# beltegeuse/rustlight

Measured on AMD Instinct MI355X. Metric: Msamples/s (paths/s) at 1080p x 128spp cbox, higher is better.
Workload: dtype f32

## Files before the change

### rustlight_amd/api.py

```python
from __future__ import annotations

import contextlib
import ctypes as C
import os
import time
from typing import Optional

import numpy as np

from . import abi
from . import scenes as S

_HERE = os.path.dirname(os.path.abspath(__file__))
LIB_PATH = os.path.join(_HERE, "lib", "librustlight_amd.so")

RL_OK = 0
RL_ERR_NO_DEVICE = -2
STRATEGY_ALL, STRATEGY_BSDF, STRATEGY_EMITTER = 0, 1, 2
STREAM_REFERENCE_ORDER, STREAM_PER_SAMPLE, STREAM_STRATIFIED = 0, 1, 2
PIPELINE_AUTO, PIPELINE_WAVEFRONT, PIPELINE_FUSED = 0, 1, 2
NUMERICS_EXACT, NUMERICS_FAST = 0, 1
LIGHT_ALL, LIGHT_SURFACE, LIGHT_VOLUME = 0, 1, 2
VPL_ALL, VPL_SURFACE, VPL_VOLUME = 0, 1, 2
LIGHT_STREAMS = ("reference", "per_path")
# ... 252 lines not shown
        for k, (w, h, rgb) in enumerate(sd.bitmaps):
            bitmaps[k].width, bitmaps[k].height, bitmaps[k].rgb = w, h, fp(rgb)
        d.bitmaps, d.n_bitmaps = bitmaps, len(sd.bitmaps)
        lights = (abi.LightDesc * max(1, len(sd.lights)))()
        for k, lt in enumerate(sd.lights):
            lights[k].kind = 0 if lt["type"] == "point" else 1
            lights[k].a = (C.c_float * 3)(*lt["a"])
            lights[k].intensity = (C.c_float * 3)(*lt["intensity"])
        d.lights, d.n_lights = lights, len(sd.lights)
        if sd.environment is not None:
            d.has_environment = 1
            d.environment_rgb = (C.c_float * 3)(*sd.environment)
        if sd.environment_map is not None:
            em = np.ascontiguousarray(sd.environment_map, np.float32); keep.append(em)
            d.env_map_width, d.env_map_height, d.env_map_rgb = em.shape[1], em.shape[0], abi.fptr(em)
        if sd.medium is not None:
            d.has_medium = 1
            d.sigma_a = (C.c_float * 3)(*sd.medium.sigma_a)
            d.sigma_s = (C.c_float * 3)(*sd.medium.sigma_s)
            d.phase_type, d.g = sd.medium.phase, sd.medium.g
        d.build_ats = int(bool(getattr(sd, "use_ats", False)))
        h = C.c_void_p()
        _check(lib().rl_scene_create_from_desc(C.byref(d), C.byref(h)))
        obj = cls.__new__(cls)
        obj.sd, obj.h = sd, h
        return obj

    @classmethod
    def load_pbrt(cls, path: str, use_shading_normals: bool = True) -> "Scene":
        h = C.c_void_p()
        _check(lib().rl_scene_load_pbrt(path.encode(), int(use_shading_normals), C.byref(h)))
        return cls(None, handle=h)

    @classmethod
    def load_mitsuba(cls, path: str, use_shading_normals: bool = True) -> "Scene":
        h = C.c_void_p()
        _check(lib().rl_scene_load_mitsuba(path.encode(), int(use_shading_normals), C.byref(h)))
        return cls(None, handle=h)

    @classmethod
    def load(cls, path: str, use_shading_normals: bool = True) -> "Scene":
        h = C.c_void_p()
        _check(lib().rl_scene_load(path.encode(), int(use_shading_normals), C.byref(h)))
        return cls(None, handle=h)

    def set_medium(self, sigma_a, sigma_s, phase=S.PHASE_ISOTROPIC, g=0.0):
        sa = np.asarray(sigma_a, dtype=np.float32)
        ss = np.asarray(sigma_s, dtype=np.float32)
        _check(lib().rl_scene_set_medium(self.h, abi.fptr(sa), abi.fptr(ss), phase, g))

    def __del__(self):
        try:
            lib().rl_scene_destroy(self.h)
        except Exception:
            pass

    @property
    def size(self):
        w, h = C.c_uint32(), C.c_uint32()
        _check(lib().rl_scene_image_size(self.h, C.byref(w), C.byref(h)))
        return w.value, h.value

    def counts(self):
        a, b, c = C.c_uint64(), C.c_uint64(), C.c_uint64()
        _check(lib().rl_scene_counts(self.h, C.byref(a), C.byref(b), C.byref(c)))
        return {"meshes": a.value, "triangles": b.value, "emitters": c.value}

    def debug_bvh(self):
        nn, npr = C.c_uint64(), C.c_uint64()
        _check(lib().rl_debug_bvh(self.h, C.byref(nn), C.byref(npr), None, None, None, None, None))
        boxes = np.zeros((nn.value, 6), np.float32)
        info = np.zeros(nn.value, np.uint64)
        count = np.zeros(nn.value, np.uint64)
        pm = np.zeros(npr.value, np.int32)
        pt = np.zeros(npr.value, np.int32)
        _check(lib().rl_debug_bvh(self.h, C.byref(nn), C.byref(npr), abi.fptr(boxes), abi.u64ptr(info), abi.u64ptr(count),
                                  pm.ctypes.data_as(C.POINTER(C.c_int32)), pt.ctypes.data_as(C.POINTER(C.c_int32))))
        return boxes, info, count, pm, pt

    def debug_emitters_cdf(self):
        n = C.c_uint64(0)
        L = lib()
        L.rl_debug_emitters_cdf.argtypes = [C.c_void_p, C.POINTER(C.c_uint64), C.POINTER(C.c_float)]
        _check(L.rl_debug_emitters_cdf(self.h, C.byref(n), None))
        out = np.zeros(n.value, np.float32)
        _check(L.rl_debug_emitters_cdf(self.h, C.byref(n), abi.fptr(out)))
        return out

    def debug_ats(self):
        L = lib()
        i32p = C.POINTER(C.c_int32)
        L.rl_debug_ats.argtypes = [C.c_void_p, C.POINTER(C.c_uint64), C.POINTER(C.c_float), C.POINTER(C.c_uint64), i32p, i32p]
        nn, nl = C.c_uint64(), C.c_uint64()
        _check(L.rl_debug_ats(self.h, C.byref(nn), None, C.byref(nl), None, None))
        nodes = np.zeros((nn.value, 16), np.float32); le = np.zeros(nl.value, np.int32); lp = np.zeros(nl.value, np.int32)
        _check(L.rl_debug_ats(self.h, C.byref(nn), abi.fptr(nodes), C.byref(nl), le.ctypes.data_as(i32p), lp.ctypes.data_as(i32p)))
        return nodes, le, lp

    def camera_ray(self, px, py):
        o = (C.c_float * 3)()
        d = (C.c_float * 3)()
        _check(lib().rl_debug_camera_ray(self.h, px, py, o, d))
        return np.array(o[:], np.float32), np.array(d[:], np.float32)


def path_params(spp=1, min_depth=0, max_depth=None, rr_depth=0, strategy=STRATEGY_ALL, single_scattering=False,
                stream_mode=STREAM_PER_SAMPLE, seed_variant=0, shard_index=0, shard_count=1, pool_slots=0, pipeline=0, sample_split=0, numerics=0) -> abi.PathParams:
    p = abi.PathParams()
    lib().rl_path_params_default(C.byref(p))
    p.spp = spp
    p.has_min_depth, p.min_depth = (0, 0) if min_depth is None else (1, min_depth)
    p.has_max_depth, p.max_depth = (0, 0) if max_depth is None else (1, max_depth)
    p.has_rr_depth, p.rr_depth = (0, 0) if rr_depth is None else (1, rr_depth)
    p.strategy = strategy
    p.single_scattering = int(single_scattering)
    p.stream_mode = stream_mode
    p.seed_variant = seed_variant
    p.shard_index, p.shard_count = shard_index, shard_count
    p.pool_slots = pool_slots
    p.pipeline = pipeline
    p.sample_split = sample_split
    p.numerics = numerics
    return p


class _ImageCalls:

    def _image_call(self, seeds, call, out=None):
        seeds = np.ascontiguousarray(seeds, dtype=np.uint64)
        st = abi.RenderStats()
        img = np.zeros((self.height, self.width, 3), dtype=np.float32) if out is None else None
        _check(call(abi.u64ptr(seeds), seeds.shape[0], abi.fptr(img) if out is None else out, C.byref(st)))
        return img, st


class Context(_ImageCalls):

    def __init__(self, scene: Scene, device: int = 0):
        self.scene = scene
        self.device = device
        h = C.c_void_p()
        _check(lib().rl_context_create(scene.h, device, C.byref(h)))
        self.h = h
        self.width, self.height = scene.size

    def close(self):
        if getattr(self, "h", None):
            lib().rl_context_destroy(self.h)
            self.h = None

    def set_option(self, name: str, value=None):
        _check(lib().rl_context_set_option(self.h, name.lower().encode(), None if value is None else str(value).encode()))

    def get_option(self, name: str):
        v = lib().rl_context_get_option(self.h, name.lower().encode())
        return None if v is None else v.decode()

    @contextlib.contextmanager
    def options(self, **kw):
        before = {k: self.get_option(k) for k in kw}
        try:
            for k, v in kw.items():
                self.set_option(k, v)
            yield self
        finally:
            for k, v in before.items():
                self.set_option(k, v)

    def __del__(self):
        try:
            self.close()
        except Exception:
            pass

    def render(self, seeds: np.ndarray, params: abi.PathParams, out_device_ptr: Optional[int] = None, stream: Optional[int] = None, out_host_ptr: Optional[int] = None):
        on_device = out_host_ptr is None and out_device_ptr is not None
        ptr = out_device_ptr if on_device else out_host_ptr
        img, st = self._image_call(seeds, lambda sp, n, out, st: lib().rl_render_path(self.h, C.byref(params), sp, n, out, int(on_device), C.c_void_p(stream) if stream else None, st),
                                   None if ptr is None else C.c_void_p(ptr))
        return img, st.as_dict()

    def _render_mc(self, fn, seeds, spp=1, stream_mode=STREAM_PER_SAMPLE, seed_variant=0, shard_index=0, shard_count=1,
                   max_distance=1.0, normal_correction=False, nb_bsdf_samples=1, nb_light_samples=1):
        p = abi.McParams()
        p.spp, p.stream_mode, p.seed_variant, p.shard_index, p.shard_count = spp, stream_mode, seed_variant, shard_index, shard_count
        p.has_max_distance, p.max_distance = (0, 0.0) if max_distance is None else (1, max_distance)
        p.normal_correction = int(normal_correction)
        p.nb_bsdf_samples, p.nb_light_samples = nb_bsdf_samples, nb_light_samples
        img, st = self._image_call(seeds, lambda sp, n, out, st: fn(self.h, C.byref(p), sp, n, out, 0, None, st))
        return img, st.as_dict()

    def render_ao(self, seeds, **kw):
        return self._render_mc(lib().rl_render_ao, seeds, **kw)

    def render_direct(self, seeds, **kw):
        return self._render_mc(lib().rl_render_direct, seeds, **kw)

    def render_light(self, seeds, spp=1, min_depth=0, max_depth=None, rr_depth=0, strategy=LIGHT_ALL, seed_variant=0, stream_mode=STREAM_PER_SAMPLE,
                     numerics=NUMERICS_EXACT, shard_count=1):
        p = path_params(spp, min_depth, max_depth, rr_depth, strategy, False, stream_mode, seed_variant, shard_count=shard_count, numerics=numerics)
        img, st = self._image_call(seeds, lambda sp, n, out, st: lib().rl_render_light(self.h, C.byref(p), sp, n, out, 0, None, st))
        d = st.as_dict()
        d["splats"], d["splats_invalid"], d["splats_saturated"] = (int(v) for v in st.reserved[:3])
        return img, d

    def vpl_generate(self, sampler: "IndependentSampler", nb_vpl=128, max_depth=None, rr_depth=0, option_vpl=VPL_ALL, streams="reference"):
        if streams not in LIGHT_STREAMS:
            raise ValueError(f"streams must be one of {LIGHT_STREAMS}, not {streams!r}")
        p = path_params(1, 0, max_depth, rr_depth, stream_mode=STREAM_REFERENCE_ORDER, seed_variant=sampler.variant)
        st = abi.RenderStats()
        h = C.c_void_p()
        fn = lib().rl_vpl_generate if streams == "reference" else lib().rl_vpl_generate_paths
        _check(fn(self.h, C.byref(p), nb_vpl, option_vpl, C.byref(sampler.s), C.byref(h), C.byref(st)))
        d = st.as_dict()
        if streams == "per_path":
            d["paths_walked"] = int(st.reserved[0])
        return VplSet(h, self), d

    def render_vpl(self, vpls: "VplSet", seeds, spp=1, option_lt=VPL_ALL, seed_variant=0, shard_index=0, shard_count=1, stream_mode=STREAM_REFERENCE_ORDER,
                   numerics=NUMERICS_EXACT):
        p = path_params(spp, 0, None, 0, stream_mode=stream_mode, seed_variant=seed_variant, shard_index=shard_index, shard_count=shard_count, numerics=numerics)
        img, st = self._image_call(seeds, lambda sp, n, out, st: lib().rl_render_vpl(self.h, vpls.h, C.byref(p), option_lt, sp, n, out, 0, None, st))
        d = st.as_dict()
        d["gather_surface"], d["gather_volume"] = int(st.reserved[0]), int(st.reserved[1])
        return img, d

    def photon_map(self, vpls: "VplSet", radius=PHOTON_RADIUS_DEFAULT, build="host"):
        if build not in TREE_BUILDS:
            raise ValueError(f"build must be one of {TREE_BUILDS}, not {build!r}")
        h = C.c_void_p()
        ms = C.c_float(0.0)
        t0 = time.perf_counter()
        if build == "device":
            _check(lib().rl_photon_map_build_device(self.h, vpls.h, radius, C.byref(h), C.byref(ms)))
        else:
            _check(lib().rl_photon_map_build(self.h, vpls.h, radius, C.byref(h)))
        m = PhotonMap(h, self)
        m.ms_build = (time.perf_counter() - t0) * 1e3
        m.ms_kernels = float(ms.value) if build == "device" else None
        return m

    def photon_tree_build_device(self, words, radius):
        w = np.ascontiguousarray(words, dtype=np.uint32).reshape(-1, VPL_WORDS)
        return _tree_arrays(lambda *out: lib().rl_photon_tree_build_device(self.h, abi.u32ptr(w), w.shape[0], radius, *out), w.shape[0])

    def _render_gather(self, fn, handle, seeds, spp, seed_variant, shard_index, shard_count, names):
        img, st = self._image_call(seeds, lambda sp, n, out, st: fn(self.h, handle, spp, seed_variant, shard_index, shard_count, sp, n, out, st))
        d = st.as_dict()
        d.update((name, int(st.reserved[k])) for k, name in enumerate(names))
        return img, d

    def render_bre(self, photons: "PhotonMap", seeds, spp=1, seed_variant=0, shard_index=0, shard_count=1):
        return self._render_gather(lib().rl_render_bre, photons.h, seeds, spp, seed_variant, shard_index, shard_count, ("nodes_entered", "photons_gathered"))

    def plane_generate(self, sampler: "IndependentSampler", nb_primitive=128, strategy="average", form="serial"):
        if form not in PLANE_FORMS:
            raise ValueError(f"form must be one of {PLANE_FORMS}, not {form!r}")
        st = abi.RenderStats()
        h = C.c_void_p()
        fn = lib().rl_plane_generate_lanes if form == "lanes" else lib().rl_plane_generate
        _check(fn(self.h, nb_primitive, plane_strategy(strategy), C.byref(sampler.s), C.byref(h), C.byref(st)))
        return PlaneSet(h, self), st.as_dict()

    def plane_map(self, planes: "PlaneSet", build="host"):
        if build not in TREE_BUILDS:
            raise ValueError(f"build must be one of {TREE_BUILDS}, not {build!r}")
        h = C.c_void_p()
        ms = C.c_float(0.0)
        t0 = time.perf_counter()
        if build == "device":
            _check(lib().rl_plane_map_build_device(self.h, planes.h, C.byref(h), C.byref(ms)))
        else:
            _check(lib().rl_plane_map_build(self.h, planes.h, C.byref(h)))
        m = PlaneMap(h, self)
        m.ms_build = (time.perf_counter() - t0) * 1e3
        m.ms_kernels = float(ms.value) if build == "device" else None
        return m

    def plane_tree_build_device(self, words):
        w = np.ascontiguousarray(words, dtype=np.uint32).reshape(-1, PLANE_WORDS)
        return _tree_arrays(lambda *out: lib().rl_plane_tree_build_device(self.h, abi.u32ptr(w), w.shape[0], *out), w.shape[0])

    def render_plane_single(self, planes: "PlaneMap", seeds, spp=1, seed_variant=0, shard_index=0, shard_count=1):
        return self._render_gather(lib().rl_render_plane_single, planes.h, seeds, spp, seed_variant, shard_index, shard_count,
                                   ("nodes_entered", "planes_intersected", "planes_visible"))

    def trace(self, origins, directions):
        o = np.ascontiguousarray(origins, dtype=np.float32).reshape(-1, 3)
        d = np.ascontiguousarray(directions, dtype=np.float32).reshape(-1, 3)
        n = o.shape[0]
        t = np.zeros(n, np.float32); u = np.zeros(n, np.float32); v = np.zeros(n, np.float32)
        m = np.zeros(n, np.int32); tr = np.zeros(n, np.int32)
        _check(lib().rl_trace_batch(self.h, n, abi.fptr(o), abi.fptr(d), abi.fptr(t), abi.fptr(u), abi.fptr(v),
                                    m.ctypes.data_as(C.POINTER(C.c_int32)), tr.ctypes.data_as(C.POINTER(C.c_int32))))
        return t, u, v, m, tr

    def trace_fast(self, origins, directions):
        o = np.ascontiguousarray(origins, dtype=np.float32).reshape(-1, 3)
        d = np.ascontiguousarray(directions, dtype=np.float32).reshape(-1, 3)
        n = o.shape[0]
        t = np.zeros(n, np.float32); m = np.zeros(n, np.int32); tr = np.zeros(n, np.int32); st = np.zeros(n, np.int32)
        i32p = C.POINTER(C.c_int32)
        fn = lib().rl_debug_trace_batch_fast
        fn.argtypes = [C.c_void_p, C.c_size_t, C.POINTER(C.c_float), C.POINTER(C.c_float), C.POINTER(C.c_float), i32p, i32p, i32p]
        _check(fn(self.h, n, abi.fptr(o), abi.fptr(d), abi.fptr(t), m.ctypes.data_as(i32p), tr.ctypes.data_as(i32p), st.ctypes.data_as(i32p)))
        return t, m, tr, st
# ... 532 lines not shown
```

### rustlight_amd/csrc/kernels/fused.hip.h

```cpp
#pragma once
#ifdef RL_STAGE_TIMERS
#include <algorithm>
#include <cstdlib>
#include <vector>
#endif

#ifndef RL_FUSED_QUEUE
#define RL_FUSED_QUEUE 0
#endif

namespace rl {

#ifdef RL_STAGE_TIMERS
__device__ unsigned long long g_stage_timers[32];
#endif
template <int MAT, bool MEDIUM, bool LDS_SCENE, int LIGHTS, int NUM, bool QUEUE = false>
__global__ void __launch_bounds__(256, LDS_SCENE ? RL_FUSED_WAVES : RL_FUSED_WAVES_STREAMING) k_path_fused(RenderConst rc_arg, DeviceScene sc_arg, StackConf stc) {
    using SMP = Rng;
#include "fused_body.inc.h"
}


template <bool LDS_SCENE>
static void launch_fused_impl(int mat, bool medium, bool area_only, dim3 grid, dim3 block, size_t lds_bytes, hipStream_t st, const RenderConst& rc, const DeviceScene& ds, const StackConf& stc) {
    with_bsdf(mat, [&](auto M) { with_flag(medium, [&](auto MED) { with_flag(area_only, [&](auto AREA) {
        constexpr int MAT = decltype(M)::value, LIGHTS = decltype(AREA)::value ? LIGHTS_AREA_ONLY : LIGHTS_ANY;
        hipLaunchKernelGGL((k_path_fused<MAT, decltype(MED)::value, LDS_SCENE, LIGHTS, RL_NUMERICS_ID, RL_FUSED_QUEUE != 0>), grid, block, lds_bytes, st, rc, ds, stc);
    }); }); });
}
template <bool LDS_SCENE>
static void dump_stage_timers_impl() {
#ifdef RL_STAGE_TIMERS
    unsigned long long h[32];
    hipMemcpyFromSymbol(h, HIP_SYMBOL(g_stage_timers), sizeof(h));
    const double tot = (double)(h[0] + h[1] + h[2] + h[3]);
    const char* names[4] = {"raygen", "extend", "shade", "shadow"};
    for (int k = 0; k < 4; k++) std::fprintf(stderr, "[stage] %-7s cycles %5.1f %%  lanes %5.1f %%\n", names[k], 100.0 * h[k] / tot, 100.0 * h[4 + k] / (double)h[8]);
    {
        const double it = (double)(h[16] + h[17] + h[18] + h[19] + h[20]), ex = it - (double)h[16], pr = (double)(h[21] + h[22] + h[23] + h[24]);
        if (it > 0) std::fprintf(stderr, "[stage] shadow stage: runs in %.1f %% of the wave-iterations; where it runs the wave holds 1-16 / 17-32 / 33-48 / 49-64 shadow rays in %.1f / %.1f / %.1f / %.1f %% (%.1f lanes on average)\n",
                                 100.0 * ex / it, 100.0 * h[17] / std::max(1.0, ex), 100.0 * h[18] / std::max(1.0, ex), 100.0 * h[19] / std::max(1.0, ex), 100.0 * h[20] / std::max(1.0, ex), (double)h[7] / std::max(1.0, ex));
        if (pr > 0) std::fprintf(stderr, "[stage] pairs of consecutive iterations: neither holds shadow rays %.1f %%, one does %.1f %%, both and <= 64 together %.1f %% (one traversal could serve both), both and > 64 %.1f %%\n",
                                 100.0 * h[21] / pr, 100.0 * h[22] / pr, 100.0 * h[23] / pr, 100.0 * h[24] / pr);
    }
    std::memset(h, 0, sizeof(h)); hipMemcpyToSymbol(HIP_SYMBOL(g_stage_timers), h, sizeof(h));
#endif
}

}
```

### rustlight_amd/csrc/kernels/fused_body.inc.h

```cpp
    const RenderConst& rc = rc_arg;
    const DeviceScene& sc = sc_arg;
    extern __shared__ __attribute__((aligned(16))) float4 smem[];
    SceneRecs recs;
    float4* after_scene = smem;
    if (LDS_SCENE) {
        stage_scene_lds(sc, smem, smem + lds_nodes_float4s(sc.n_nodes));
        recs.nodes = smem; recs.tris = smem + lds_nodes_float4s(sc.n_nodes);
        after_scene = smem + lds_scene_float4s(sc.n_nodes, sc.n_prims);
    } else {
        recs.nodes = streamed_nodes<TravStackT<false>>(sc);
        recs.tris = reinterpret_cast<const float4*>(sc.tris);
    }
    const unsigned tid = blockIdx.x * blockDim.x + threadIdx.x;
    unsigned long long* cold_q = reinterpret_cast<unsigned long long*>(after_scene);
    float* cold_f = reinterpret_cast<float*>(cold_q + 256 * FusedState::kColdQ);
    unsigned* cold_u = reinterpret_cast<unsigned*>(cold_f + 256 * FusedState::kColdF);
    const TravStackT<LDS_SCENE> stack(make_stack<LDS_SCENE>(stc, cold_u + 256 * FusedState::kColdU, tid));
    FusedState ps;
    ps.cold_q = cold_q + threadIdx.x; ps.cold_f = cold_f + threadIdx.x; ps.cold_u = cold_u + threadIdx.x;
#pragma unroll
    for (int i = 0; i < F_COUNT; i++) ps.fv[i] = 0.0f;
#pragma unroll
    for (int i = 0; i < U_COUNT; i++) ps.uv[i] = 0u;
#pragma unroll
    for (int i = 0; i < Q_COUNT; i++) ps.qv[i] = 0ull;
    storec(ps, F_AR, czero());
    PU(U_CURSOR) = 0u; PU(U_SAMPLE) = 0u;
    const unsigned item0 = (tid & ((1u << rc.item_shift) - 1u)) == 0u ? (tid >> rc.item_shift) : 0xffffffffu;
    PU(U_ITEM) = item0;
    PU(U_PRIM) = 0xffffffffu;
    PU(U_FLAGS) = item0 < rc.n_items ? (ST_REGEN | ST_FRESH) : ST_FINISHED;
    unsigned n_samples = 0, n_draws = 0, n_vertices = 0, n_shadow = 0, n_ext = 0;
#ifdef RL_STAGE_TIMERS
    unsigned long long tm[4] = {0, 0, 0, 0}, ln[5] = {0, 0, 0, 0, 0};
    unsigned long long sh_hist[5] = {0, 0, 0, 0, 0}, sh_pair[4] = {0, 0, 0, 0}, sh_cyc_exec = 0; unsigned sh_prev = 0, sh_parity = 0;
#define RL_T0 { t0 = __builtin_readcyclecounter(); }
#define RL_T1(K, COND) { unsigned long long t1 = __builtin_readcyclecounter(); tm[K] += t1 - t0; ln[K] += __popcll(__ballot(COND)); t0 = t1; }
    unsigned long long t0;
#else
#define RL_T0
#define RL_T1(K, COND)
#endif
    constexpr bool qmode = QUEUE;
    constexpr unsigned kQDone = 0xffffffffu;
    if constexpr (qmode) {
        PU(U_ITEM) = 0u;
        PU(U_FLAGS) = ST_FINISHED;
    }
    for (;;) {
    if constexpr (qmode) {
        const char __attribute__((address_space(4)))* kq = (const char __attribute__((address_space(4)))*)__builtin_amdgcn_kernarg_segment_ptr();
        asm volatile("" : "+s"(kq));
        const RenderConst& rc_arg = *(const RenderConst*)kq;
        const unsigned ipb = 256u * rc_arg.split, total = rc_arg.q_n * ipb;
        unsigned fl = PU(U_FLAGS);
        for (int tries = 0; tries < 4; tries++) {
            if ((fl & ST_FINISHED) && PU(U_ITEM) != kQDone) {
                const unsigned c = atomicAdd(rc_arg.q_ctr, 1u);
                if (c >= total) PU(U_ITEM) = kQDone;
                else {
                    const unsigned j = rc_arg.q_list[c / ipb], idx = c - (c / ipb) * ipb;
                    unsigned bx_, by_, bw_, bh_;
                    block_geometry(rc_arg, rc_arg.owned_blocks[j], &bx_, &by_, &bw_, &bh_);
                    const unsigned npx = min(rc_arg.cursor_end, bw_ * bh_) - min(rc_arg.cursor_begin, bw_ * bh_);
                    if (idx < npx * rc_arg.split) {
                        PU(U_ITEM) = rc_arg.block_item_base[j] * rc_arg.split + idx;
                        PU(U_PRIM) = 0xffffffffu; PU(U_CURSOR) = 0u; PU(U_SAMPLE) = 0u;
                        storec(ps, F_AR, czero());
                        fl = ST_REGEN | ST_FRESH;
                    }
                }
            }
            if (__ballot((fl & ST_FINISHED) && PU(U_ITEM) != kQDone) == 0ull) break;
        }
        PU(U_FLAGS) = fl;
        if (__ballot(!(fl & ST_FINISHED)) == 0ull) {
            if (__ballot((fl & ST_FINISHED) && PU(U_ITEM) != kQDone) == 0ull) break;
            continue;
        }
    }
    if (!(PU(U_FLAGS) & ST_FINISHED)) do {
        const char __attribute__((address_space(4)))* ka = (const char __attribute__((address_space(4)))*)__builtin_amdgcn_kernarg_segment_ptr();
        asm volatile("" : "+s"(ka));
        constexpr size_t sc_off = (sizeof(RenderConst) + alignof(DeviceScene) - 1) / alignof(DeviceScene) * alignof(DeviceScene);
        static_assert(sc_off == offsetof(PathKernargs, sc) && offsetof(PathKernargs, rc) == 0, "kernarg layout of k_path_fused(RenderConst, DeviceScene, StackConf)");
        const DeviceScene& sc = *(const DeviceScene*)(ka + sc_off);
        const RenderConst& rc = MEDIUM ? *(const RenderConst*)ka : rc_arg;
        RL_T0
#ifdef RL_STAGE_TIMERS
        ln[4] += 64;
        const bool c0 = PU(U_FLAGS) & ST_REGEN;
#endif
        if (PU(U_FLAGS) & ST_REGEN) raygen_slot<true, decltype(ps), SMP>(rc, sc, ps, n_samples, n_draws);
        RL_T1(0, c0)
#ifdef RL_STAGE_TIMERS
        const bool c1 = PU(U_FLAGS) & ST_RAY;
#endif
        if (PU(U_FLAGS) & ST_RAY) {
            extend_slot(sc, recs, stack, ps);
            RL_T1(1, c1)
            shade_slot<MAT, MEDIUM, LIGHTS, false, SMP>(rc, sc, ps, PU(U_FLAGS), n_vertices, n_draws, n_shadow, n_ext);
        }
        RL_T1(2, c1)
#ifdef RL_STAGE_TIMERS
        const bool c3 = PU(U_FLAGS) & ST_SHADOW;
#endif
        if (PU(U_FLAGS) & ST_SHADOW) shadow_slot(sc, recs, stack, ps);
#ifdef RL_STAGE_TIMERS
        { const unsigned nsh = (unsigned)__popcll(__ballot(c3)); sh_hist[nsh == 0u ? 0 : 1 + (nsh - 1u) / 16u]++;
          if (nsh) sh_cyc_exec += __builtin_readcyclecounter() - t0;
          if (sh_parity) { const unsigned a = sh_prev, b = nsh; sh_pair[(a == 0u && b == 0u) ? 0 : ((a == 0u || b == 0u) ? 1 : (a + b <= 64u ? 2 : 3))]++; }
          sh_prev = nsh; sh_parity ^= 1u; }
#endif
        RL_T1(3, c3)
    } while (!qmode && !(PU(U_FLAGS) & ST_FINISHED));
    if (!qmode) break;
    }
#ifdef RL_STAGE_TIMERS
    if ((threadIdx.x & 63u) == 0u) { for (int k = 0; k < 4; k++) { atomicAdd(&g_stage_timers[k], tm[k]); atomicAdd(&g_stage_timers[4 + k], ln[k]); } atomicAdd(&g_stage_timers[8], ln[4]);
        for (int k = 0; k < 5; k++) atomicAdd(&g_stage_timers[16 + k], sh_hist[k]); for (int k = 0; k < 4; k++) atomicAdd(&g_stage_timers[21 + k], sh_pair[k]); atomicAdd(&g_stage_timers[25], sh_cyc_exec); }
#endif
    {
        const int which[5] = {STAT_SAMPLES, STAT_VERTICES, STAT_DRAWS, STAT_SHADOW_RAYS, STAT_EXT_RAYS};
        const unsigned vals[5] = {n_samples, n_vertices, n_draws, n_shadow, n_ext};
        block_stats<5>(rc.partials, which, vals);
    }
```

### rustlight_amd/csrc/kernels/knobs.h

```cpp
#pragma once
#include <cstdlib>
#include <cstring>
#include <string>

namespace rl {

enum KnobId {
    K_REF_SINGLE_PASS,
    K_STATE_BUDGET_MB,
    K_NO_OVERLAP,
    K_CHAIN_SERIAL,
    K_CHAIN_NO_PRE,
    K_CHAIN_NO_TREELETS,
    K_SPEC_FORCE,
    K_SPEC_DRAWS_PER_SAMPLE,
    K_ITEM_SHIFT,
    K_FUSED_DYNAMIC,
    K_EVAL_SPLIT,
    K_EVAL_MIN, K_EVAL_DIV,
    K_NO_EVENTS,
    K_QUEUE_DEBUG,
    K_SPEC_GROUP, K_SPEC_SUB, K_SPEC_CAP, K_SPEC_PROBE, K_SPEC_LEAD, K_SPEC_LEAD_MAX, K_SPEC_LEAD_VAR, K_SPEC_EXTRA, K_SPEC_DENSE, K_SPEC_DENSE_FRAC,
    K_SPEC_PROBE_EVERY, K_SPEC_KS, K_SPEC_KE, K_SPEC_SERIAL_RATIO, K_SPEC_NO_TRIVIAL, K_SPEC_LDS_LIMIT_TEST, K_SPEC_STATS, K_SPEC_WAVE_TIMES,
    K_SPEC_LDS_LEVELS,
    K_VPL_BATCH_PATHS,
    K_PHOTON_TREE_GROUP_PHOTONS,
    K_PLANE_GENERATE_LANES,
    K_PLANE_TREE_DEVICE,
    K_PLANE_TREE_GROUP_PLANES,
    K_FORCE_STREAMING,
    K_GENERIC_LIGHTS,
    K_COUNT
};

struct Knobs {
    struct Entry { bool set = false; std::string value; };
    Entry e[K_COUNT];

    static const char* name_of(int k) {
        static const char* const names[K_COUNT] = {
            "ref_single_pass", "state_budget_mb", "no_overlap", "chain_serial", "chain_no_pre", "chain_no_treelets", "spec_force", "spec_draws_per_sample", "item_shift",
            "fused_dynamic", "eval_split", "eval_min", "eval_div", "no_events", "queue_debug",
            "spec_group", "spec_sub", "spec_cap", "spec_probe", "spec_lead", "spec_lead_max", "spec_lead_var", "spec_extra", "spec_dense", "spec_dense_frac",
            "spec_probe_every", "spec_ks", "spec_ke", "spec_serial_ratio", "spec_no_trivial", "spec_lds_limit_test", "spec_stats", "spec_wave_times", "spec_lds_levels", "vpl_batch_paths", "photon_tree_group_photons",
            "plane_generate_lanes", "plane_tree_device", "plane_tree_group_planes",
            "force_streaming", "generic_lights"};
        return names[k];
    }
    static int find(const char* name) {
        if (!name) return -1;
        for (int k = 0; k < K_COUNT; k++) if (std::strcmp(name, name_of(k)) == 0) return k;
        return -1;
    }
    void from_environment() {
        for (int k = 0; k < K_COUNT; k++) {
            std::string env = "RL_";
            for (const char* p = name_of(k); *p; p++) env += (char)((*p >= 'a' && *p <= 'z') ? *p - 'a' + 'A' : *p);
            const char* v = std::getenv(env.c_str());
            e[k].set = v != nullptr;
            e[k].value = v ? v : "";
        }
    }
    bool has(int k) const { return e[k].set; }
    const char* str(int k) const { return e[k].set ? e[k].value.c_str() : nullptr; }
    long long i(int k, long long dflt) const { return e[k].set ? std::atoll(e[k].value.c_str()) : dflt; }
    double f(int k, double dflt) const { return e[k].set ? std::atof(e[k].value.c_str()) : dflt; }
};

}
```

### rustlight_amd/csrc/kernels/path_render.hip.h

```cpp
#pragma once

namespace {

using namespace rl;

struct Plan { unsigned split, n_items, P, item_shift; };
struct Chunk { unsigned c0, c1, n_pix; std::vector<unsigned> base; };

class PathRender : RenderFrame {
public:
    PathRender(rl_context* c, const rl_path_params* p, const uint64_t* seeds, size_t nb, float* out, int out_dev, void* stream_arg, rl_render_stats* s)
        : RenderFrame(c, seeds, nb, out, out_dev, stream_arg, s, p->shard_index, p->shard_count), params(p) {}

    int run() {
        int r;
        if ((r = choose_form()) != RL_OK) return r;
        plan_chunks();
        if ((r = plan_lanes()) != RL_OK) return r;
        if ((r = upload()) != RL_OK) return r;
        if (two_pass) r = run_two_pass();
        else if (fused) r = run_fused();
        else r = run_wavefront();
        if (r != RL_OK) return r;
        return finish();
    }

private:
    const rl_path_params* const params;
    bool per_sample = false, fused = false, fast_math = false, two_pass = false, medium = false;
    bool strat = false;
    bool overlap_wanted = false;
    bool one_lane_per_pixel = false;
    bool overlapped = false;
    size_t state_budget = 0;
    std::vector<Chunk> chunks;
    unsigned max_chunk_pix = 0;
    Plan plan{1u, 0u, 0u, 0u}, plan_chain{1u, 0u, 0u, 0u};
    unsigned split = 1, n_items = 0, item_shift = 0, P = 0, n_item_pixels = 0;
    Pool pool{};
    RenderConst rc{};
    StackConf stc{};
    size_t lds_trav = 0, lds_fused = 0;
    double ms[4] = {0, 0, 0, 0}, ms_fused = 0.0, ms_chain = 0.0, ms_eval_span = 0.0;
    uint64_t iterations = 0, launches = 2, n_extend = 0;
    unsigned long long spec_stat[3] = {0, 0, 0};
    unsigned spec_group = 0;
    bool spec = false;
    SpecConf spc{};
    unsigned spec_threads = 0;
    StackConf stc_c{}, stc_s{};
    size_t lds_chain = 0, lds_spec = 0;
    int spec_levels = -1;

    static constexpr unsigned kMaxEvalLaunches = 256u;
    static constexpr size_t kEventsPerIter = 8;

    int choose_form() {
        strat = params->stream_mode == RL_STREAM_STRATIFIED;
        per_sample = params->stream_mode == RL_STREAM_PER_SAMPLE || strat;
        if (params->pipeline > 2) { rl_set_error("pipeline must be 0 (auto), 1 (wavefront) or 2 (fused)"); return RL_ERR_INVALID_ARGUMENT; }
        fused = params->pipeline == 2 || (params->pipeline == 0 && params->pool_slots == 0);
        fast_math = params->numerics == RL_NUMERICS_FAST;
        if (fast_math && !fused) { rl_set_error("numerics = fast exists for the persistent kernel only (pipeline 0 or 2, pool_slots 0)"); return RL_ERR_UNSUPPORTED; }
        if (fast_math && strat) { rl_set_error("numerics = fast is not built with the stratified sampler (stream_mode = RL_STREAM_STRATIFIED)"); return RL_ERR_UNSUPPORTED; }
        medium = ctx->ds.medium.enabled != 0;
        two_pass = !per_sample && fused && !owned.empty() && !knobs.has(K_REF_SINGLE_PASS);
        state_budget = max_state_bytes();
        if (two_pass && (size_t)owned.size() * params->spp * 32 > state_budget) two_pass = false;
        return RL_OK;
    }

    Plan plan_items(bool per_pixel, unsigned n_pix, unsigned n_chains) const {
        Plan pl{1u, 0u, 0u, 0u};
        if (per_pixel && n_pix > 0) {
            const unsigned fused_groups = (n_pix + 255u) / 256u;
            const unsigned fused_auto = fused_groups >= 6000u ? 1u : std::max(1u, 16384u / std::max(1u, fused_groups));
            unsigned want = params->sample_split ? params->sample_split
                                : (fused ? (ctx->lds_scene ? fused_auto : std::max(fused_auto, 64u))
                                         : (ctx->lds_scene ? 1u : std::max(1u, (8u << 20) / std::max(1u, n_pix))));
            if (overlap_wanted && !params->sample_split) want = std::max(want, (unsigned)std::max<long long>(1, knobs.i(K_EVAL_SPLIT, 4)));
            pl.split = std::max(1u, std::min(want, params->spp));
            if ((size_t)n_pix * params->spp * 3 * sizeof(float) > kSampleBufBudget || one_lane_per_pixel) pl.split = 1;
            while (pl.split > 1 && (size_t)n_pix * pl.split > (size_t)0x7fffff00u) pl.split--;
        }
        pl.n_items = per_pixel ? n_pix * pl.split : n_chains;
        unsigned Pp = params->pool_slots ? std::min(params->pool_slots, std::max(pl.n_items, 1u)) : std::min<unsigned>(pl.n_items, 16u << 20);
        Pp = std::max(256u, (unsigned)(((unsigned long long)Pp + 255ull) / 256ull * 256ull));
        if (fused) {
            const unsigned resident = (unsigned)cus * (unsigned)(ctx->lds_scene ? RL_FUSED_WAVES : RL_FUSED_WAVES_STREAMING) * 256u;
            const bool dynamic_items = knobs.has(K_FUSED_DYNAMIC) ? knobs.i(K_FUSED_DYNAMIC, 0) != 0 : (medium || !ctx->lds_scene);
            Pp = std::max(256u, (std::min(pl.n_items, dynamic_items ? resident : pl.n_items) + 255u) / 256u * 256u);
            const unsigned resident4 = (unsigned)cus * 4u * 256u / ((medium && !per_pixel) ? 2u : 1u);
            while (pl.item_shift < 6u && ((size_t)pl.n_items << (pl.item_shift + 1u)) <= resident4) pl.item_shift++;
            if (!per_pixel && knobs.has(K_ITEM_SHIFT)) pl.item_shift = std::min(6u, (unsigned)std::max<long long>(0, knobs.i(K_ITEM_SHIFT, 0)));
            if (pl.item_shift) Pp = std::max(256u, (unsigned)((((size_t)pl.n_items << pl.item_shift) + 255u) / 256u * 256u));
        }
        pl.P = Pp;
        return pl;
    }

    void plan_chunks() {
        if (two_pass && !knobs.has(K_STATE_BUDGET_MB)) {
            size_t free_b = 0, total_b = 0;
            if (hipMemGetInfo(&free_b, &total_b) == hipSuccess) state_budget = std::min(state_budget, ctx->d_sample_states.capacity() * sizeof(unsigned long long) + free_b / 10 * 6);
            else (void)hipGetLastError();
        }
        for (bool planned_states = false; two_pass && !planned_states;) {
            const size_t budget = state_budget;
            const size_t per_cursor = (size_t)owned.size() * params->spp * 32;
            if (per_cursor > budget) { two_pass = false; chunks.clear(); break; }
            chunks.clear();
            const unsigned cursors_per_chunk = (unsigned)std::max<size_t>(1, std::min<size_t>(256, budget / std::max<size_t>(1, per_cursor)));
            for (unsigned c0 = 0; c0 < 256u; c0 += cursors_per_chunk) {
                Chunk ch; ch.c0 = c0; ch.c1 = std::min(256u, c0 + cursors_per_chunk); ch.n_pix = 0;
                for (size_t j = 0; j < owned.size(); j++) {
                    const BlockRect r = block_rect(owned[j], nby, W, H);
                    const unsigned npx = r.w * r.h;
                    ch.base.push_back(ch.n_pix);
                    ch.n_pix += std::min(ch.c1, npx) - std::min(ch.c0, npx);
                }
                if (ch.n_pix) chunks.push_back(std::move(ch));
            }
            size_t need = 0;
            for (const Chunk& ch : chunks) need = std::max(need, (size_t)ch.n_pix * params->spp * 4);
            if (ctx->d_sample_states.ensure(need) == RL_OK) planned_states = true;
            else state_budget /= 2;
        }
        max_chunk_pix = 0;
        for (const Chunk& ch : chunks) max_chunk_pix = std::max(max_chunk_pix, ch.n_pix);
    }

    int plan_lanes() {
        overlap_wanted = two_pass && ctx->stream2 && !fast_math && !knobs.has(K_NO_OVERLAP) && knobs.i(K_SPEC_GROUP, 0) != 256;
        int rcode;
        for (int attempt = 0; attempt < 2; attempt++) {
            plan = two_pass ? plan_items(true, max_chunk_pix, 0) : plan_items(per_sample, n_pixels, (unsigned)owned.size());
            if (two_pass) for (const Chunk& ch : chunks) { const Plan pc = plan_items(true, ch.n_pix, 0); plan.P = std::max(plan.P, pc.P); plan.split = std::max(plan.split, pc.split); }
            plan_chain = two_pass ? plan_items(false, 0, (unsigned)owned.size()) : Plan{1u, 0u, 0u, 0u};
            split = plan.split; n_items = plan.n_items; item_shift = plan.item_shift;
            P = std::max(plan.P, plan_chain.P);
            n_item_pixels = two_pass ? max_chunk_pix : n_pixels;
            if (split <= 1) break;
            if (ctx->d_sample_buf.ensure((size_t)n_item_pixels * params->spp * 3) == RL_OK) break;
            if (params->sample_split || attempt == 1) return RL_ERR_HIP;
            one_lane_per_pixel = true; overlap_wanted = false;
        }
        if ((rcode = alloc_tables()) != RL_OK) return rcode;
        if (per_sample || two_pass) {
            if (per_sample && (rcode = ctx->d_item_seed.ensure(n_item_pixels)) != RL_OK) return rcode;
            if ((rcode = ctx->d_item_pixel.ensure(n_item_pixels)) != RL_OK) return rcode;
        }
        if (two_pass) {
            if ((rcode = ctx->d_sample_states.ensure((size_t)max_chunk_pix * params->spp * 4)) != RL_OK) return rcode;
            if ((rcode = ctx->d_chain_states.ensure(owned.size() * 4)) != RL_OK) return rcode;
        }
        if (!fused && ctx->pool_q.capacity() / Q_COUNT < P) {
            ctx->pool_f.reset(); ctx->pool_u.reset(); ctx->pool_q.reset();
            if (ctx->pool_f.ensure((size_t)F_COUNT * P) != RL_OK || ctx->pool_u.ensure((size_t)U_COUNT * P) != RL_OK || ctx->pool_q.ensure((size_t)Q_COUNT * P) != RL_OK) {
                ctx->pool_f.reset(); ctx->pool_u.reset(); ctx->pool_q.reset();
                rl_set_error("out of device memory for a path-state pool of " + std::to_string(P) + " slots");
                return RL_ERR_HIP;
            }
        }
        pool = Pool{ctx->pool_f.get(), ctx->pool_u.get(), ctx->pool_q.get(), P};
        return alloc_output(std::max<size_t>((P + 255) / 256, (size_t)cus * 8u * rl_context::kEvalStreams));
    }

    int upload() {
        int rcode;
        if ((rcode = RenderFrame::upload(!two_pass, true)) != RL_OK) return rcode;
        Counters init{};
        init.active = std::min(plan.P, n_items);
        init.next_item = item_shift ? n_items : plan.P;
        if (!two_pass) HIP_OK(hipMemcpyAsync(ctx->d_counters.get(), &init, sizeof(init), hipMemcpyHostToDevice, st));
        if ((rcode = zero_rows()) != RL_OK) return rcode;

        rc = render_const(params->spp, params->stream_mode, params->seed_variant);
        rc.has_min = params->has_min_depth; rc.min_depth = params->min_depth;
        rc.has_max = params->has_max_depth; rc.max_depth = params->max_depth;
        rc.has_rr = params->has_rr_depth; rc.rr_depth = params->rr_depth;
        rc.strategy = params->strategy; rc.single_scattering = params->single_scattering;
        rc.n_items = n_items;
        rc.item_shift = item_shift;
        rc.split = split; rc.sample_buf = ctx->d_sample_buf.get();
        rc.sample_states = ctx->d_sample_states.get(); rc.chain_states = ctx->d_chain_states.get();

        lds_trav = traversal_lds_bytes(ctx, ctx->lds_scene, 256, true);
        if ((rcode = stack_conf(ctx, (size_t)((P + 255) / 256) * 256, &stc)) != RL_OK) return rcode;
        lds_fused = traversal_lds_bytes(ctx, ctx->lds_scene, 256, false) + kFusedColdBytes;

        const dim3 block(256);
        if (per_sample && !owned.empty()) hipLaunchKernelGGL(k_seed_pixels, dim3(((unsigned)owned.size() + 63) / 64), dim3(64), 0, st, rc);
        if (!fused) hipLaunchKernelGGL(k_init, dim3((plan.P + 255) / 256), block, 0, st, rc, pool);

        return grow_events(kEventsPerIter * (per_sample ? 8u : 32u));
    }

    void launch_fused(const RenderConst& rcl, dim3 grid, hipStream_t on, const StackConf* stcl = nullptr) const {
        const int mat = ctx->single_bsdf ? ctx->bsdf_type : -1;
        const StackConf& s = stcl ? *stcl : stc;
        if (strat)
            (ctx->lds_scene ? launch_fused_strat_lds : launch_fused_strat_stream)(medium, ctx->area_lights_only, grid, dim3(256), lds_fused, on, rcl, ctx->ds, s);
        else if (rcl.queue_mode != 0u)
            (ctx->lds_scene ? launch_fusedq_lds : launch_fusedq_stream)(mat, medium, ctx->area_lights_only, grid, dim3(256), lds_fused, on, rcl, ctx->ds, s);
        else
            (ctx->lds_scene ? (fast_math ? launch_fused_lds_fast : launch_fused_lds) : (fast_math ? launch_fused_stream_fast : launch_fused_stream))(mat, medium, ctx->area_lights_only, grid, dim3(256), lds_fused, on, rcl, ctx->ds, s);
    }

    void drain() const {
        (void)hipStreamSynchronize(st);
        for (int k = 0; k < rl_context::kEvalStreams; k++) if (ctx->eval_streams[k]) (void)hipStreamSynchronize(ctx->eval_streams[k]);
        (void)hipGetLastError();
    }
    struct DrainOnError {
        const PathRender* r; bool armed = true;
        ~DrainOnError() { if (armed) r->drain(); }
    };

    int plan_chain_pass() {
        stc_c = stc;
        if (ctx->lds_scene && !medium && ctx->ds.n_nodes <= 64u && ctx->ds.n_prims <= 64u && plan_chain.item_shift >= 5u && !knobs.has(K_CHAIN_NO_PRE)) stc_c.pre_group = 1 << plan_chain.item_shift;
        const bool treelets = !ctx->lds_scene && !fast_math && ctx->ds.nodes_t && ctx->ds.root_t >= 0 && plan_chain.item_shift >= 5u && ctx->ds.stack_depth <= 512u && !knobs.has(K_CHAIN_NO_TREELETS);
        if (treelets) stc_c.pre_group = 1 << plan_chain.item_shift;
        auto chain_lds_of = [&](bool tl) {
            return traversal_lds_bytes(ctx, ctx->lds_scene, 256, false) + (tl ? (size_t)(256 / stc_c.pre_group) * (72 + (ctx->ds.stack_depth + 1) / 2) * 16
                   : (stc_c.pre_group ? (size_t)(256 / stc_c.pre_group) * ((size_t)ctx->ds.n_nodes * 32 + (size_t)ctx->ds.n_prims * 8) : 0));
        };
        if (chain_lds_of(treelets) > ctx->lds_limit) stc_c.pre_group = 0;
        lds_chain = chain_lds_of(treelets && stc_c.pre_group != 0);

        spec = !fast_math && !knobs.has(K_CHAIN_SERIAL);
        const bool spec_force = knobs.has(K_SPEC_FORCE);
        if (spec && !spec_force) {
            const double nbar = knobs.f(K_SPEC_DRAWS_PER_SAMPLE, medium ? 150.0 : 12.0);
            if ((double)params->spp < 4.0 * nbar) spec = false;
        }
        spec_levels = ctx->lds_scene ? -1 : (int)std::max<long long>(0, std::min<long long>(knobs.i(K_SPEC_LDS_LEVELS, kSpecLdsLevelsStreaming), lds_levels_of(ctx)));
        lds_spec = traversal_lds_bytes(ctx, ctx->lds_scene, 256, false, spec_levels) + (size_t)(kSpecColdWords - (ctx->lds_scene ? 0 : kSpecHelperWords)) * 256 * 4 + kSpecGroupLdsBytes;
        const size_t spec_lds_limit = knobs.has(K_SPEC_LDS_LIMIT_TEST) ? (size_t)knobs.i(K_SPEC_LDS_LIMIT_TEST, 0) : ctx->lds_limit;
        if (lds_spec > spec_lds_limit) spec = false;
        spc = SpecConf{};
        spec_threads = 0;
        if (spec) {
            unsigned group = 16u;
            while (group < 64u && (size_t)owned.size() * group < (size_t)cus * 4u * 2u * 64u) group <<= 1;
            if (!ctx->lds_scene) group = 64u;
            if (knobs.has(K_SPEC_GROUP)) { const long long g = knobs.i(K_SPEC_GROUP, 0); if (g == 16 || g == 32 || g == 64 || g == 256) group = (unsigned)g; }
            spc.group = group;
            spc.sub = std::max(1u, group / 16u);
            spc.serial_ratio = spec_force ? 0.0f : (float)knobs.f(K_SPEC_SERIAL_RATIO, 3.0);
            if (knobs.has(K_SPEC_SUB)) { const long long v = knobs.i(K_SPEC_SUB, 0); if ((v == 1 || v == 2 || v == 4 || v == 8 || v == 16) && (unsigned)v <= group) spc.sub = (unsigned)v; }
            spc.cap = std::max(96u, std::min(3u * params->spp + 64u, 1u << 20));
            if (knobs.has(K_SPEC_CAP)) spc.cap = std::max(4u, (unsigned)knobs.i(K_SPEC_CAP, 0));
            spc.probe = knobs.has(K_SPEC_PROBE) ? (unsigned)knobs.i(K_SPEC_PROBE, 0) : std::min(32u, std::max(4u, params->spp));
            spc.lead = (unsigned)knobs.i(K_SPEC_LEAD, 24);
            spc.lead_max = (unsigned)knobs.i(K_SPEC_LEAD_MAX, 128);
            spc.lead_var = (float)knobs.f(K_SPEC_LEAD_VAR, 100.0);
            spc.extra = (unsigned)knobs.i(K_SPEC_EXTRA, 0);
            spc.dense = !ctx->lds_scene ? 0u : (knobs.has(K_SPEC_DENSE) ? std::min(64u, (unsigned)knobs.i(K_SPEC_DENSE, 0)) : 16u);
            spc.dense_frac = (float)knobs.f(K_SPEC_DENSE_FRAC, 0.6);
            spc.probe_every = (unsigned)knobs.i(K_SPEC_PROBE_EVERY, 0);
            spc.ks = (float)knobs.f(K_SPEC_KS, group >= 64u ? 2.5 : 1.65);
            spc.ke = (float)knobs.f(K_SPEC_KE, group >= 64u ? 2.5 : 1.65);
            spec_threads = (unsigned)((((size_t)owned.size() * group) + 255u) / 256u * 256u);
            const size_t need = (size_t)spec_threads * spc.cap * 36u;
            size_t free_b = 0, total_b = 0;
            const size_t have = ctx->d_trk_off.capacity() * 4u + ctx->d_trk_st.capacity() * 16u;
            if (hipMemGetInfo(&free_b, &total_b) != hipSuccess) { (void)hipGetLastError(); free_b = 0; }
            if (need > have && need - have > free_b / 2u) spec = false;
            if (spec && (ctx->d_trk_off.ensure((size_t)spec_threads * spc.cap) != RL_OK || ctx->d_trk_st.ensure((size_t)spec_threads * spc.cap * 2u) != RL_OK)) spec = false;
        }
        int rcode;
        if (spec) {
            const bool expand = !params->has_max_depth || 1u < params->max_depth;
            const bool no_trivial = knobs.has(K_SPEC_NO_TRIVIAL);
            const uint64_t key = ((uint64_t)params->shard_index << 33) | ((uint64_t)shard_count << 1) | (expand ? 1u : 0u);
            if (key != ctx->trivial_key || ctx->d_trivial.capacity() < owned.size() * 8 || no_trivial) {
                std::vector<unsigned> masks;
                trivial_pixel_masks(trivial_input(ctx), params, owned, nby, no_trivial, &masks);
                if ((rcode = ctx->d_trivial.ensure(masks.size())) != RL_OK) return rcode;
                HIP_OK(hipMemcpyAsync(ctx->d_trivial.get(), masks.data(), masks.size() * sizeof(unsigned), hipMemcpyHostToDevice, st));
                HIP_OK(hipStreamSynchronize(st));
                ctx->trivial_key = no_trivial ? ~0ull : key;
            }
            if ((rcode = ctx->d_spec_stats.ensure(32 + 8 * (size_t)(spec_threads / 64u))) != RL_OK) return rcode;
            HIP_OK(hipMemsetAsync(ctx->d_spec_stats.get(), 0, 32 * sizeof(unsigned long long), st));
            spc.trk_off = ctx->d_trk_off.get(); spc.trk_st = ctx->d_trk_st.get(); spc.trivial = ctx->d_trivial.get();
            spc.stats = (stats || knobs.has(K_SPEC_STATS)) ? ctx->d_spec_stats.get() : nullptr;
            const size_t n_thr = std::max<size_t>((size_t)((P + 255) / 256) * 256, spec_threads);
            if ((rcode = stack_conf(ctx, n_thr, &stc_s, false, spec_levels)) != RL_OK) return rcode;
            if ((rcode = stack_conf(ctx, n_thr, &stc)) != RL_OK) return rcode;
            stc_c.overflow = stc.overflow; stc_c.overflow_stride = stc.overflow_stride;
        }
        return RL_OK;
    }

    void launch_chain_pass(const RenderConst& ra) const {
        const int mat = ctx->single_bsdf ? ctx->bsdf_type : -1;
        if (spec) (ctx->lds_scene ? launch_spec_lds : launch_spec_stream)(mat, medium, dim3(spec_threads / 256u), dim3(256), lds_spec, st, ra, ctx->ds, stc_s, spc);
        else (ctx->lds_scene ? (fast_math ? launch_chain_lds_fast : launch_chain_lds) : (fast_math ? launch_chain_stream_fast : launch_chain_stream))(mat, medium, dim3((plan_chain.P + 255) / 256), dim3(256), lds_chain, st, ra, ctx->ds, stc_c);
    }

    int prepare_queue(RenderConst& ra, unsigned chain_grid) {
        const size_t n_dev = 16 + (size_t)kMaxEvalLaunches + owned.size(), n_flags = 16 + owned.size();
        int rcode;
        if ((rcode = ctx->d_queue.ensure(n_dev)) != RL_OK || (rcode = ctx->h_flags.ensure(n_flags)) != RL_OK || (rcode = ctx->h_list.ensure(owned.size())) != RL_OK) return rcode;
        HIP_OK(hipMemsetAsync(ctx->d_queue.get(), 0, (16 + (size_t)kMaxEvalLaunches) * sizeof(unsigned), st));
        ra.queue = ctx->d_queue.get(); ra.chain_grid = chain_grid;
        ra.done_flags = ctx->h_flags.device_ptr() + 16; ra.started_flag = ctx->h_flags.device_ptr();
        ra.queue_seq = ++ctx->queue_seq;
        if (ra.queue_seq == 0u) { std::memset(ctx->h_flags.get(), 0, ctx->h_flags.capacity() * sizeof(unsigned)); ra.queue_seq = ++ctx->queue_seq; }
        return RL_OK;
    }

    int overlap_loop(const RenderConst& rb, const Plan& pb, unsigned seq, dim3 grid_q, const StackConf& stc_q) {
        HIP_OK(hipEventRecord(ctx->ev_chain_done, st));
        const unsigned n_blocks_owned = (unsigned)owned.size();
        volatile unsigned* hf = ctx->h_flags.get();
        std::vector<unsigned> waiting(n_blocks_owned);
        for (unsigned j = 0; j < n_blocks_owned; j++) waiting[j] = j;
        unsigned n_listed = 0, n_launches = 0, scan_from = 0;
        const auto poll_us = std::chrono::microseconds(50 + n_blocks_owned / 100u);
        bool chain_over = false, started = false;
        const unsigned resident = grid_q.x;
        const unsigned batch_min = (unsigned)std::max<long long>(1, knobs.i(K_EVAL_MIN, 64)), batch_div = (unsigned)std::max<long long>(1, knobs.i(K_EVAL_DIV, 5));
        std::chrono::steady_clock::time_point t_first{};
        auto launch_batch = [&](unsigned first, unsigned count) -> int {
            const unsigned k = n_launches % (unsigned)rl_context::kEvalStreams;
            hipStream_t on = ctx->eval_streams[k];
            HIP_OK(hipMemcpyAsync(ctx->d_queue.get() + 16 + kMaxEvalLaunches + first, ctx->h_list.get() + first, count * sizeof(unsigned), hipMemcpyHostToDevice, on));
            RenderConst rq = rb;
            rq.q_list = ctx->d_queue.get() + 16 + kMaxEvalLaunches + first; rq.q_n = count; rq.q_ctr = ctx->d_queue.get() + 16 + n_launches;
            rq.partials = rb.partials + (size_t)k * resident * STAT_COUNT;
            StackConf stc_k = stc_q;
            if (stc_k.overflow) stc_k.overflow += (size_t)k * resident * 256u * 2u;
            const unsigned wgs = std::min<unsigned>(resident, (unsigned)(((size_t)count * 256u * pb.split + 255u) / 256u));
            if (n_launches == 0) t_first = std::chrono::steady_clock::now();
// ... 56 lines not shown
        cinit.next_item = pb.item_shift ? pb.n_items : pb.P;
        if (overlap) cinit.next_item = pb.n_items;
        HIP_OK(hipMemcpyAsync(ctx->d_counters.get(), &cinit, sizeof(cinit), hipMemcpyHostToDevice, st));
        const dim3 grid_q((unsigned)cus * (unsigned)(ctx->lds_scene ? RL_FUSED_WAVES : RL_FUSED_WAVES_STREAMING));
        StackConf stc_q = stc;
        if (overlap && (rcode = stack_conf(ctx, (size_t)grid_q.x * 256 * rl_context::kEvalStreams, &stc_q, true)) != RL_OK) return rcode;
        if (timing) hipEventRecord(ctx->events[0], st);
        launch_chain_pass(ra);
        if (timing) hipEventRecord(ctx->events[1], st);
        HIP_OK(hipGetLastError());
        if (overlap) {
            rb.queue = ctx->d_queue.get(); rb.queue_mode = 1u; rb.chain_grid = chain_grid;
            if ((rcode = overlap_loop(rb, pb, ra.queue_seq, grid_q, stc_q)) != RL_OK) return rcode;
            overlapped = true;
            if (timing) hipEventRecord(ctx->events[3], st);
        } else {
            if (timing) hipEventRecord(ctx->events[2], st);
            launch_fused(rb, dim3((pb.P + 255) / 256), st);
            if (timing) hipEventRecord(ctx->events[3], st);
        }
        if (pb.split > 1) hipLaunchKernelGGL(k_fold_samples, dim3((ch.n_pix + 255) / 256), block, 0, st, rb);
        HIP_OK(hipGetLastError());
        HIP_OK(hipStreamSynchronize(st));
        guard.armed = false;
        if (timing) {
            float t = 0.0f;
            HIP_OK(hipEventElapsedTime(&t, ctx->events[0], ctx->events[1])); ms_chain += t;
            HIP_OK(hipEventElapsedTime(&t, ctx->events[overlap ? 1 : 2], ctx->events[3])); ms_fused += t;
            if (!overlap) ms_eval_span += t;
        }
        launches += 3 + (pb.split > 1 ? 1 : 0);
        return RL_OK;
    }

    int run_two_pass() {
        int rcode;
        if ((rcode = plan_chain_pass()) != RL_OK) return rcode;
        for (const Chunk& ch : chunks) if ((rcode = run_chunk(ch)) != RL_OK) return rcode;
        dump_stage_timers(ctx->lds_scene);
        if (ctx->lds_scene) dump_chain_timers_lds(); else dump_chain_timers_stream();
        if (spec && spc.stats && (rcode = read_spec_stats()) != RL_OK) return rcode;
        iterations = chunks.size();
        return RL_OK;
    }

    int read_spec_stats() {
        unsigned long long spec_totals[32] = {0};
        HIP_OK(hipMemcpy(spec_totals, ctx->d_spec_stats.get(), sizeof(spec_totals), hipMemcpyDeviceToHost));
        spec_group = spc.group; spec_stat[0] = spec_totals[0]; spec_stat[1] = spec_totals[1]; spec_stat[2] = spec_totals[2];
        const bool verbose = knobs.has(K_SPEC_STATS);
        if (verbose) std::fprintf(stderr, "[spec] LDS per workgroup %zu bytes (scene %zu, %d stack levels)\n", lds_spec, (size_t)(ctx->lds_scene ? ctx->scene_lds_bytes : 0), stc_s.lds_levels);
        if (verbose) std::fprintf(stderr, "[spec] group %u x sub %u cap %u: %llu speculative + %llu serial + %llu probe samples for %llu camera samples (%.2f x, %.2f serial per pixel), %llu wave iterations\n",
            spc.group, spc.sub, spc.cap, spec_totals[0], spec_totals[1], spec_totals[2], (unsigned long long)n_pixels * params->spp,
            (double)(spec_totals[0] + spec_totals[1] + spec_totals[2]) / std::max(1.0, (double)n_pixels * params->spp), (double)spec_totals[1] / std::max(1u, n_pixels), spec_totals[3]);
        if (knobs.has(K_SPEC_WAVE_TIMES) && spec_totals[8]) {
            std::vector<unsigned long long> wt(8 * (size_t)(spec_threads / 64u));
            HIP_OK(hipMemcpy(wt.data(), ctx->d_spec_stats.get() + 32, wt.size() * 8, hipMemcpyDeviceToHost));
            FILE* f = std::fopen(knobs.str(K_SPEC_WAVE_TIMES), "w");
            if (f) { unsigned long long t0 = ~0ull; for (size_t w = 0; w < wt.size() / 8; w++) if (wt[8 * w]) t0 = std::min(t0, wt[8 * w]);
                     for (size_t w = 0; w < wt.size() / 8; w++) std::fprintf(f, "%zu %.3f %.3f %llu %llu %.3f %.3f %llu %llu\n", w, (wt[8 * w] - t0) * 1e-5, (wt[8 * w + 1] - t0) * 1e-5, wt[8 * w + 2], wt[8 * w + 3], wt[8 * w + 4] * 1e-5, wt[8 * w + 5] * 1e-5, wt[8 * w + 6], wt[8 * w + 7]); std::fclose(f); }
        }
        if (verbose && spec_totals[8]) {
            const double tot = (double)(spec_totals[4] + spec_totals[5] + spec_totals[6] + spec_totals[7] + spec_totals[8]);
            std::fprintf(stderr, "[spec] cycles: bookkeeping %.1f %%, plan %.1f %%, thread %.1f %%, copy-out %.1f %%, extend+shade %.1f %%; %.1f lanes per traced iteration, %.1f %% of the traced iterations serial only, %.0f cycles per wave iteration\n",
                100.0 * spec_totals[4] / tot, 100.0 * spec_totals[5] / tot, 100.0 * spec_totals[6] / tot, 100.0 * spec_totals[7] / tot, 100.0 * spec_totals[8] / tot,
                (double)spec_totals[9] / std::max<double>(1.0, (double)spec_totals[10]), 100.0 * spec_totals[11] / std::max<double>(1.0, (double)spec_totals[10]), tot / std::max<double>(1.0, (double)spec_totals[3]));
            { const double ts = (double)(spec_totals[16] + spec_totals[17] + spec_totals[18] + spec_totals[19] + spec_totals[20]);
              std::fprintf(stderr, "[spec] iterations after a serial-only one (%.1f %% of all cycles): bookkeeping %.1f %%, plan %.1f %%, thread %.1f %%, copy-out %.1f %%, extend+shade %.1f %%\n", 100.0 * ts / tot,
                100.0 * spec_totals[16] / ts, 100.0 * spec_totals[17] / ts, 100.0 * spec_totals[18] / ts, 100.0 * spec_totals[19] / ts, 100.0 * spec_totals[20] / ts); }
            std::fprintf(stderr, "[spec] slow walks: %llu from a pixel's start, %llu across a missing link, %llu past the last track\n", spec_totals[12], spec_totals[13], spec_totals[14]);
            std::fprintf(stderr, "[spec] serial walks on helpers: %llu (one lane: %llu), %llu rounds, %llu samples taken from them\n", spec_totals[26], spec_totals[27], spec_totals[24], spec_totals[25]);
        }
        return RL_OK;
    }

    int run_fused() {
        if (timing) hipEventRecord(ctx->events[0], st);
        launch_fused(rc, dim3((plan.P + 255) / 256), st);
        if (timing) hipEventRecord(ctx->events[1], st);
        HIP_OK(hipGetLastError());
        HIP_OK(hipStreamSynchronize(st));
        if (timing) { float t = 0.0f; HIP_OK(hipEventElapsedTime(&t, ctx->events[0], ctx->events[1])); ms_fused = t; ms_eval_span = t; }
        dump_stage_timers(ctx->lds_scene);
        launches += 1;
        iterations = 1;
        return RL_OK;
    }

    int run_wavefront() {
        const dim3 block(256);
        const dim3 grid_all((plan.P + 255) / 256);
        const bool use_sort = !ctx->single_bsdf;
        const unsigned sort_chunks = split > 1 ? 4u : 1u;
        const dim3 grid_sort((P + 1023) / 1024);
        const dim3 grid_persistent(std::min<unsigned>((P + 255) / 256, (unsigned)cus * 8u));
        const unsigned poll_every = per_sample ? 8u : 32u;
        const DeviceScene& ds = ctx->ds;
        unsigned in_batch = 0;
        auto flush_events = [&](unsigned count) -> int {
            for (unsigned i = 0; i < count; i++)
                for (int k = 0; k < 4; k++) {
                    float t = 0.0f;
                    HIP_OK(hipEventElapsedTime(&t, ctx->events[kEventsPerIter * i + 2 * k], ctx->events[kEventsPerIter * i + 2 * k + 1]));
                    ms[k] += t;
                }
            return RL_OK;
        };
        for (;;) {
            hipEvent_t* ev = timing ? &ctx->events[kEventsPerIter * in_batch] : nullptr;
            if (timing) hipEventRecord(ev[0], st);
            if (strat) launch_raygen_strat(grid_persistent, block, st, rc, ds, pool);
            else hipLaunchKernelGGL(k_raygen, grid_persistent, block, 0, st, rc, ds, pool);
            if (timing) { hipEventRecord(ev[1], st); hipEventRecord(ev[2], st); }
            if (ctx->lds_scene) hipLaunchKernelGGL((k_extend<true>), grid_all, block, lds_trav, st, rc, ds, pool, stc);
            else hipLaunchKernelGGL((k_extend<false>), grid_all, block, lds_trav, st, rc, ds, pool, stc);
            if (timing) { hipEventRecord(ev[3], st); hipEventRecord(ev[4], st); }
            if (strat) launch_shade_sorted_strat(medium, sort_chunks, sort_chunks == 4u ? grid_sort : grid_all, block, st, rc, ds, pool);
            else if (use_sort) launch_shade_sorted(medium, sort_chunks, sort_chunks == 4u ? grid_sort : grid_all, block, st, rc, ds, pool);
            else launch_shade_type(ctx->bsdf_type, medium, grid_all, block, st, rc, ds, pool);
            launches += 1;
            if (timing) { hipEventRecord(ev[5], st); hipEventRecord(ev[6], st); }
            if (ctx->lds_scene) hipLaunchKernelGGL((k_shadow<true>), grid_all, block, lds_trav, st, rc, ds, pool, stc);
            else hipLaunchKernelGGL((k_shadow<false>), grid_all, block, lds_trav, st, rc, ds, pool, stc);
            if (timing) hipEventRecord(ev[7], st);
            launches += 3;
            n_extend++;
            iterations++;
            in_batch++;
            if (in_batch == poll_every) {
                HIP_OK(hipGetLastError());
                HIP_OK(hipMemcpyAsync(ctx->h_counters.get(), ctx->d_counters.get(), sizeof(Counters), hipMemcpyDeviceToHost, st));
                HIP_OK(hipStreamSynchronize(st));
                if (timing) { int r = flush_events(in_batch); if (r != RL_OK) return r; }
                in_batch = 0;
                if (ctx->h_counters.get()->active == 0) break;
            }
            if (iterations > (uint64_t)1 << 28) { rl_set_error("render did not terminate"); return RL_ERR_HIP; }
        }
#ifdef RL_TRAV_STATS
        {
            unsigned long long h[8];
            HIP_OK(hipStreamSynchronize(st));
            hipMemcpyFromSymbol(h, HIP_SYMBOL(g_trav_stats), sizeof(h));
            std::fprintf(stderr, "[trav] rays %llu (zero-step %.1f %%)  steps/ray %.1f  tris/ray %.1f  waves %llu  lanes/wave %.1f  paid steps/ray %.1f  step utilisation %.1f %%\n",
                         h[0], 100.0 * h[5] / (double)h[0], (double)h[1] / h[0], (double)h[2] / h[0], h[4], (double)h[0] / h[4], (double)h[3] / h[0], 100.0 * h[1] / (double)h[3]);
            std::memset(h, 0, sizeof(h)); hipMemcpyToSymbol(HIP_SYMBOL(g_trav_stats), h, sizeof(h));
        }
#endif
        return RL_OK;
    }

    int finish() {
        if (split > 1 && !two_pass) { hipLaunchKernelGGL(k_fold_samples, dim3((n_pixels + 255) / 256), dim3(256), 0, st, rc); launches += 1; }
        const int rcode = download();
        if (rcode != RL_OK) return rcode;
        if (stats) {
            stats->iterations = iterations;
            stats->kernel_launches = launches;
            stats->ms_raygen = ms[0]; stats->ms_extend = ms[1]; stats->ms_shade = ms[2]; stats->ms_shadow = ms[3];
            stats->ms_other = ms_fused;
            stats->ms_prepass = ms_chain;
            stats->n_extend_launches = n_extend;
            stats->reserved[0] = spec_stat[0]; stats->reserved[1] = spec_stat[1]; stats->reserved[2] = spec_stat[2]; stats->reserved[3] = spec_group;
            stats->chunks = two_pass ? (uint32_t)chunks.size() : 0u;
            stats->overlapped = overlapped ? 1u : 0u;
            stats->ms_eval_span = ms_eval_span;
        }
        return RL_OK;
    }
};

}
```

### rustlight_amd/csrc/kernels/pathstate.hip.h

```cpp
#pragma once

namespace rl {

enum FField {
    F_OX, F_OY, F_OZ, F_DX, F_DY, F_DZ,
    F_T, F_U, F_V,
    F_BR, F_BG, F_BB,
    F_TR, F_TG, F_TB,
    F_LR, F_LG, F_LB,
    F_AR, F_AG, F_AB,
    F_WR, F_WG, F_WB,
    F_RR, F_PDF,
    F_SX, F_SY, F_SZ,
    F_CR, F_CG, F_CB,
    F_XI,
    F_COUNT
};
enum UField { U_FLAGS, U_DEPTH, U_PRIM, U_ITEM, U_CURSOR, U_SAMPLE, U_COUNT };
enum QField { Q_R0, Q_R1, Q_R2, Q_R3, Q_I0, Q_I1, Q_I2, Q_I3, Q_COUNT };

enum : unsigned {
    ST_FINISHED = 1u,
    ST_REGEN = 2u,
    ST_FRESH = 4u,
    ST_RAY = 8u,
    ST_SHADOW = 16u,
    ST_PREV_SHIFT = 5u,
    ST_PDF_SA = 128u,
    ST_ZEROED = 256u,
};
enum : unsigned { PREV_SENSOR = 0u, PREV_SURFACE = 1u, PREV_SURFACE_SMOOTH = 2u, PREV_VOLUME = 3u };

#ifndef RL_FUSED_WAVES
#define RL_FUSED_WAVES 4
#endif
#ifndef RL_FUSED_WAVES_STREAMING
#define RL_FUSED_WAVES_STREAMING 6
#endif
static constexpr unsigned kDepthCap = 2048u;

struct Pool {
    float* f;
    unsigned* u;
    unsigned long long* q;
    unsigned P;
};

struct Counters {
    unsigned int active;
    unsigned int next_item;
    unsigned int pad[2];
};

static constexpr int kLdsStackLevels = 12;
static constexpr size_t kSampleBufBudget = (size_t)16 << 30;
struct StackConf { int lds_levels; int* overflow; size_t overflow_stride; int pre_group; };

#ifndef RL_SPEC_LDS_LEVELS_STREAMING
#define RL_SPEC_LDS_LEVELS_STREAMING 4
#endif
static constexpr int kSpecLdsLevelsStreaming = RL_SPEC_LDS_LEVELS_STREAMING;
static constexpr int kSpecColdWords = 30;
static constexpr int kSpecHelperWords = 2;
static constexpr size_t kSpecGroupLdsBytes = (256 / 16) * 32 + 64 + (256 / 16) * 64 + (256 / 16) * 16;
struct SpecConf {
    unsigned group;
    unsigned sub;
    unsigned cap;
    unsigned probe;
    unsigned lead;
    unsigned lead_max; float lead_var;
    unsigned extra;
    unsigned probe_every;
    unsigned dense; float dense_frac;
    float serial_ratio;
    float ks, ke;
    unsigned* trk_off;
    ulonglong2* trk_st;
    const unsigned* trivial;
    unsigned long long* stats;
};

template <bool LDS_ONLY = false>
RL_DEV TravStackT<LDS_ONLY> make_stack(const StackConf& sc_, unsigned* lds_after_list, size_t global_thread) {
    TravStackT<LDS_ONLY> st;
    st.lds = (typename TravStackT<LDS_ONLY>::LdsPtr)(lds_after_list) + threadIdx.x;
    st.lds_levels = sc_.lds_levels;
    st.glob = sc_.overflow ? (typename TravStackT<LDS_ONLY>::GlobPtr)(sc_.overflow) + global_thread : nullptr;
    st.glob_stride = sc_.overflow_stride;
    return st;
}

struct RenderConst {
    unsigned spp;
    int has_min, has_max, has_rr;
    unsigned min_depth, max_depth, rr_depth;
    int strategy, single_scattering;
    int stream_mode, seed_variant;
    float inv_spp;
    unsigned W, H, nby;
    unsigned n_items;
    unsigned item_shift;
    unsigned split;
    float* sample_buf;
    const unsigned* owned_blocks;
    const unsigned* block_item_base;
    unsigned n_owned;
    const unsigned long long* block_seeds;
    unsigned long long* item_seed;
    unsigned* item_pixel;
    float* out;
    Counters* counters;
    unsigned long long* partials;
    unsigned long long* sample_states;
    unsigned n_state_pixels;
    unsigned cursor_begin, cursor_end;
    unsigned long long* chain_states;
    unsigned* queue;
    unsigned* done_flags;
    unsigned* started_flag;
    unsigned queue_seq, chain_grid;
    unsigned queue_mode;
    const unsigned* q_list;
    unsigned q_n;
    unsigned* q_ctr;
};
RL_DEV void queue_workgroup_started(const RenderConst& rc) {
    if (atomicAdd(rc.queue, 1u) + 1u == rc.chain_grid) __hip_atomic_store(rc.started_flag, rc.queue_seq, __ATOMIC_RELEASE, __HIP_MEMORY_SCOPE_SYSTEM);
}
RL_DEV void queue_push(const RenderConst& rc, unsigned item) {
    __builtin_amdgcn_fence(__ATOMIC_RELEASE, "agent");
    __hip_atomic_store(&rc.done_flags[item], rc.queue_seq, __ATOMIC_RELEASE, __HIP_MEMORY_SCOPE_SYSTEM);
}
enum : int { kStreamGivenStates = 1000 };

struct PathKernargs { RenderConst rc; DeviceScene sc; StackConf stc; };
struct SpecKernargs { RenderConst rc; DeviceScene sc; StackConf stc; SpecConf spec; };

struct PoolState {
    Pool pool; unsigned slot;
    RL_DEV float& f(int field) const { return pool.f[(size_t)field * pool.P + slot]; }
    RL_DEV unsigned& u(int field) const { return pool.u[(size_t)field * pool.P + slot]; }
    RL_DEV unsigned long long& q(int field) const { return pool.q[(size_t)field * pool.P + slot]; }
};
struct RegState {
    float fv[F_COUNT]; unsigned uv[U_COUNT]; unsigned long long qv[Q_COUNT];
    RL_DEV float& f(int field) { return fv[field]; }
    RL_DEV unsigned& u(int field) { return uv[field]; }
    RL_DEV unsigned long long& q(int field) { return qv[field]; }
};
struct FusedState {
    float fv[F_COUNT]; unsigned uv[U_COUNT]; unsigned long long qv[Q_COUNT];
    float* cold_f; unsigned* cold_u; unsigned long long* cold_q;
    static constexpr int kColdF = 3, kColdU = 3, kColdQ = 4;
    RL_DEV float& f(int field) { return (field >= F_AR && field <= F_AB) ? cold_f[(field - F_AR) * 256] : fv[field]; }
    RL_DEV unsigned& u(int field) { return (field >= U_ITEM && field <= U_SAMPLE) ? cold_u[(field - U_ITEM) * 256] : uv[field]; }
    RL_DEV unsigned long long& q(int field) { return (field >= Q_I0) ? cold_q[(field - Q_I0) * 256] : qv[field]; }
};
static constexpr size_t kFusedColdBytes = 256 * (FusedState::kColdQ * 8 + FusedState::kColdF * 4 + FusedState::kColdU * 4);
#define PF(field) ps.f(field)
#define PU(field) ps.u(field)
#define PQ(field) ps.q(field)

template <class PS> RL_DEV V3 load3(PS& ps, int f0) { return mk3(PF(f0), PF(f0 + 1), PF(f0 + 2)); }
template <class PS> RL_DEV Col loadc(PS& ps, int f0) { return mkc(PF(f0), PF(f0 + 1), PF(f0 + 2)); }
template <class PS> RL_DEV void store3(PS& ps, int f0, V3 v) { PF(f0) = v.x; PF(f0 + 1) = v.y; PF(f0 + 2) = v.z; }
template <class PS> RL_DEV void storec(PS& ps, int f0, Col c) { PF(f0) = c.r; PF(f0 + 1) = c.g; PF(f0 + 2) = c.b; }
template <class PS> RL_DEV Rng load_rng(PS& ps, int q0) { Rng r; r.s0 = PQ(q0); r.s1 = PQ(q0 + 1); r.s2 = PQ(q0 + 2); r.s3 = PQ(q0 + 3); return r; }
template <class PS> RL_DEV void store_rng(PS& ps, int q0, const Rng& r) { PQ(q0) = r.s0; PQ(q0 + 1) = r.s1; PQ(q0 + 2) = r.s2; PQ(q0 + 3) = r.s3; }

enum { STAT_SAMPLES, STAT_VERTICES, STAT_EXT_RAYS, STAT_SHADOW_RAYS, STAT_DRAWS, STAT_COUNT = 8 };
RL_DEV unsigned wave_sum(unsigned v) {
    for (int off = 32; off > 0; off >>= 1) v += __shfl_down(v, off, 64);
    return v;
}
template <int N>
RL_DEV void block_stats(unsigned long long* partials, const int (&which)[N], const unsigned (&vals)[N]) {
    __shared__ unsigned s_acc[N];
    if (threadIdx.x < N) s_acc[threadIdx.x] = 0u;
    __syncthreads();
#pragma unroll
    for (int k = 0; k < N; k++) {
        unsigned v = wave_sum(vals[k]);
        if ((threadIdx.x & 63u) == 0u && v) atomicAdd(&s_acc[k], v);
    }
    __syncthreads();
    if (threadIdx.x < N && s_acc[threadIdx.x]) partials[(size_t)blockIdx.x * STAT_COUNT + which[threadIdx.x]] += s_acc[threadIdx.x];
}

RL_DEV unsigned block_compact(bool pred, unsigned slot, unsigned* list) {
    const unsigned lane = threadIdx.x & 63u, wave = threadIdx.x >> 6;
    const unsigned long long mask = __ballot(pred);
    const unsigned rank = __popcll(mask & ((1ull << lane) - 1ull));
    unsigned* wave_cnt = list + 256;
    if (lane == 0u) wave_cnt[wave] = (unsigned)__popcll(mask);
    __syncthreads();
    unsigned base = 0, total = 0;
#pragma unroll
    for (unsigned w = 0; w < 4u; w++) { unsigned c = wave_cnt[w]; if (w < wave) base += c; total += c; }
    if (pred) list[base + rank] = slot;
    __syncthreads();
    return total;
}

RL_DEV void block_geometry(const RenderConst& rc, unsigned b, unsigned* bx, unsigned* by, unsigned* bw, unsigned* bh) {
    *bx = (b / rc.nby) * 16u;
    *by = (b % rc.nby) * 16u;
    *bw = min(16u, rc.W - *bx);
    *bh = min(16u, rc.H - *by);
}

}
```

### rustlight_amd/csrc/kernels/stages.hip.h

```cpp
#pragma once

namespace rl {

RL_DEV V3 camera_direction(const DeviceScene& sc, float u, float v) {
    const float* m = sc.camera.sample_to_camera;
    float sx = div_rn(u, (float)sc.camera.width), sy = div_rn(v, (float)sc.camera.height), sz = 0.0f;
    float hx = ((m[0] * sx + m[4] * sy) + m[8] * sz) + m[12] * 1.0f;
    float hy = ((m[1] * sx + m[5] * sy) + m[9] * sz) + m[13] * 1.0f;
    float hz = ((m[2] * sx + m[6] * sy) + m[10] * sz) + m[14] * 1.0f;
    float hw = ((m[3] * sx + m[7] * sy) + m[11] * sz) + m[15] * 1.0f;
    float inv_w = div_rn(1.0f, hw);
    V3 near_p = mk3(hx * inv_w, hy * inv_w, hz * inv_w);
    V3 dl = normalize(near_p);
    const float* tw = sc.camera.to_world;
    return mk3(((tw[0] * dl.x + tw[4] * dl.y) + tw[8] * dl.z) + tw[12] * 0.0f,
               ((tw[1] * dl.x + tw[5] * dl.y) + tw[9] * dl.z) + tw[13] * 0.0f,
               ((tw[2] * dl.x + tw[6] * dl.y) + tw[10] * dl.z) + tw[14] * 0.0f);
}

RL_DEV Rng load_sample_state(const RenderConst& rc, unsigned s, unsigned p) {
    const ulonglong2* q = reinterpret_cast<const ulonglong2*>(rc.sample_states + 4 * ((size_t)s * rc.n_state_pixels + p));
    const ulonglong2 a = q[0], b = q[1];
    Rng r; r.s0 = a.x; r.s1 = a.y; r.s2 = b.x; r.s3 = b.y;
    return r;
}
RL_DEV void store_sample_state(const RenderConst& rc, unsigned s, unsigned p, const Rng& r) {
    ulonglong2* q = reinterpret_cast<ulonglong2*>(rc.sample_states + 4 * ((size_t)s * rc.n_state_pixels + p));
    q[0] = make_ulonglong2(r.s0, r.s1); q[1] = make_ulonglong2(r.s2, r.s3);
}

template <class PS>
RL_DEV void raygen_chain_slot(const RenderConst& rc, const DeviceScene& sc, PS& ps) {
    const unsigned flags = PU(U_FLAGS);
    const unsigned item = PU(U_ITEM);
    unsigned s = PU(U_SAMPLE), cursor = PU(U_CURSOR);
    unsigned bx, by, bw, bh;
    const unsigned b = rc.owned_blocks[item];
    block_geometry(rc, b, &bx, &by, &bw, &bh);
    const unsigned c_end = min(rc.cursor_end, bw * bh);
    Rng rng;
    if (flags & ST_FRESH) {
        cursor = rc.cursor_begin; s = 0;
        if (cursor >= c_end) { if (rc.queue) queue_push(rc, item); PU(U_FLAGS) = ST_FINISHED; return; }
        if (rc.cursor_begin == 0u) rng = rng_seed(rc.block_seeds[b], rc.seed_variant);
        else { const unsigned long long* q = rc.chain_states + 4 * (size_t)item; rng.s0 = q[0]; rng.s1 = q[1]; rng.s2 = q[2]; rng.s3 = q[3]; }
    } else {
        rng = load_rng(ps, Q_R0);
        s++;
        if (s == rc.spp) { s = 0; cursor++; }
        if (cursor == c_end) {
            unsigned long long* q = rc.chain_states + 4 * (size_t)item;
            q[0] = rng.s0; q[1] = rng.s1; q[2] = rng.s2; q[3] = rng.s3;
            if (rc.queue) queue_push(rc, item);
            PU(U_FLAGS) = ST_FINISHED;
            return;
        }
    }
    store_sample_state(rc, s, rc.block_item_base[item] + (cursor - rc.cursor_begin), rng);
    const unsigned px = bx + cursor % bw, py = by + cursor / bw;
    const float u = (float)px + rng_next_f32(rng);
    const float v = (float)py + rng_next_f32(rng);
    PU(U_SAMPLE) = s;
    PU(U_CURSOR) = cursor;
    const bool expand = (!rc.has_max || 1u < rc.max_depth);
    if (!expand) { store_rng(ps, Q_R0, rng); PU(U_FLAGS) = ST_REGEN; return; }
    store3(ps, F_DX, camera_direction(sc, u, v));
    if (sc.medium.enabled) PF(F_XI) = rng_next_f32(rng);
    store_rng(ps, Q_R0, rng);
    PU(U_DEPTH) = 1u;
    PU(U_FLAGS) = ST_RAY | (PREV_SENSOR << ST_PREV_SHIFT) | ST_PDF_SA;
}

template <bool DYNAMIC, class PS, class SMP = Rng>
RL_DEV void raygen_slot(const RenderConst& rc, const DeviceScene& sc, PS& ps, unsigned& n_samples, unsigned& n_draws) {
    unsigned flags = PU(U_FLAGS);
    if (!(flags & ST_REGEN)) return;
    const bool fresh = (flags & ST_FRESH) != 0u;
    unsigned item = PU(U_ITEM), s = PU(U_SAMPLE), cursor = PU(U_CURSOR);
    Col acc = loadc(ps, F_AR);
    bool need_item = fresh;
    unsigned bx = 0, by = 0, bw = 1, bh = 1;
    if (rc.stream_mode == RL_STREAM_REFERENCE_ORDER && item < rc.n_items) block_geometry(rc, rc.owned_blocks[item], &bx, &by, &bw, &bh);
    constexpr bool STRAT = !std::is_same<SMP, Rng>::value;
    const bool per_pixel = STRAT || rc.stream_mode != RL_STREAM_REFERENCE_ORDER;
    const bool given = !STRAT && rc.stream_mode == kStreamGivenStates;
    const unsigned split = per_pixel ? rc.split : 1u;
    const unsigned pitem = split > 1u ? item / split : item;
    if (!fresh && split > 1u) {
        const Col L = loadc(ps, F_LR);
        float* dst = rc.sample_buf + 3 * ((size_t)s * (rc.n_items / split) + pitem);
        dst[0] = L.r; dst[1] = L.g; dst[2] = L.b;
        s += split;
        if (s >= rc.spp) need_item = true;
    } else if (!fresh) {
        acc = acc + loadc(ps, F_LR);
        s++;
        if (s == rc.spp) {
            unsigned pix = per_pixel ? rc.item_pixel[item] : (by + cursor / bw) * rc.W + (bx + cursor % bw);
            Col px = scale_unguarded(acc, rc.inv_spp);
            rc.out[3 * (size_t)pix] = px.r; rc.out[3 * (size_t)pix + 1] = px.g; rc.out[3 * (size_t)pix + 2] = px.b;
            acc = czero();
            s = 0;
            if (per_pixel) need_item = true;
            else { cursor++; if (cursor == bw * bh) need_item = true; }
        }
    }
    Rng rng;
    if (need_item) {
        if (!fresh) item = DYNAMIC ? atomicAdd(&rc.counters->next_item, 1u) : rc.n_items;
        if (item >= rc.n_items) {
            PU(U_FLAGS) = ST_FINISHED;
            if (DYNAMIC) atomicSub(&rc.counters->active, 1u);
            return;
        }
        cursor = 0;
        if (given) {
            const unsigned pi = split > 1u ? item / split : item;
            if (split > 1u) s = item % split;
            rng = load_sample_state(rc, s, pi);
        } else if (per_pixel) {
            const unsigned pi = split > 1u ? item / split : item;
            Rng item_rng = rng_seed(rc.item_seed[pi], rc.seed_variant);
            if (split > 1u) { s = item % split; for (unsigned k = 0; k < s; k++) rng_next_u64(item_rng); }
            rng = rng_seed(rng_next_u64(item_rng), rc.seed_variant);
            store_rng(ps, Q_I0, item_rng);
        } else {
            unsigned b = rc.owned_blocks[item];
            block_geometry(rc, b, &bx, &by, &bw, &bh);
            rng = rng_seed(rc.block_seeds[b], rc.seed_variant);
        }
        PU(U_ITEM) = item;
    } else if (given) {
        rng = load_sample_state(rc, s, pitem);
    } else if (per_pixel) {
        Rng item_rng = load_rng(ps, Q_I0);
        for (unsigned k = 1; k < split; k++) rng_next_u64(item_rng);
        rng = rng_seed(rng_next_u64(item_rng), rc.seed_variant);
        store_rng(ps, Q_I0, item_rng);
    } else {
        rng = load_rng(ps, Q_R0);
    }
    unsigned px, py;
    if (per_pixel) { unsigned pix = rc.item_pixel[split > 1u ? item / split : item]; px = pix % rc.W; py = pix / rc.W; }
    else { px = bx + cursor % bw; py = by + cursor / bw; }
    SMP smp = SmpState<SMP>::begin(rc, rng, split > 1u ? item / split : item, s);
    float u = (float)px + smp_next(smp);
    float v = (float)py + smp_next(smp);
    n_draws += 2;
    n_samples++;
    storec(ps, F_AR, acc);
    PU(U_SAMPLE) = s;
    PU(U_CURSOR) = cursor;
    const bool expand = (!rc.has_max || 1u < rc.max_depth);
    if (!expand) {
        storec(ps, F_LR, czero());
        smp_store(ps, smp);
        PU(U_FLAGS) = ST_REGEN;
        return;
    }
    const V3 d = camera_direction(sc, u, v);
    store3(ps, F_DX, d);
    if (sc.medium.enabled) { PF(F_XI) = smp_next(smp); n_draws++; }
    smp_store(ps, smp);
    PU(U_DEPTH) = 1u;
    PU(U_FLAGS) = ST_RAY | (PREV_SENSOR << ST_PREV_SHIFT) | ST_PDF_SA | smp_flag_bits(smp);
}

template <bool LDS_SCENE>
RL_DEV TravStackT<LDS_SCENE> open_scene(const DeviceScene& sc, const StackConf& stc, float4* smem, unsigned tid, SceneRecs* recs) {
    float4* after_scene = smem;
    if (LDS_SCENE) {
        stage_scene_lds(sc, smem, smem + lds_nodes_float4s(sc.n_nodes));
        recs->nodes = smem; recs->tris = smem + lds_nodes_float4s(sc.n_nodes);
        after_scene = smem + lds_scene_float4s(sc.n_nodes, sc.n_prims);
    } else {
        recs->nodes = streamed_nodes<TravStackT<false>>(sc);
        recs->tris = reinterpret_cast<const float4*>(sc.tris);
    }
    return make_stack<LDS_SCENE>(stc, reinterpret_cast<unsigned*>(after_scene), tid);
}

template <class PS, class Stack>
RL_DEV void extend_slot(const DeviceScene& sc, const SceneRecs& recs, const Stack& stack, PS& ps, int* dbg = nullptr) {
    const unsigned flags = PU(U_FLAGS);
    const bool primary = ((flags >> ST_PREV_SHIFT) & 3u) == PREV_SENSOR;
    V3 o = primary ? mk3(sc.camera.position[0], sc.camera.position[1], sc.camera.position[2]) : load3(ps, F_OX);
    V3 d = load3(ps, F_DX);
    Hit hit; hit.t = kF32Max; hit.u = 0.0f; hit.v = 0.0f; hit.prim = -1;
    traverse<false>(recs, Stack::kBvh4 ? sc.root4 : sc.root, mk3(sc.root_min[0], sc.root_min[1], sc.root_min[2]), mk3(sc.root_max[0], sc.root_max[1], sc.root_max[2]),
                    o, d, kEps, kF32Max, hit, stack);
    PF(F_T) = hit.t; PF(F_U) = hit.u; PF(F_V) = hit.v;
    PU(U_PRIM) = (unsigned)hit.prim;
    if (dbg) { dbg[0] = hit.steps; dbg[1] = hit.tris; }
}
template <class Stack>
RL_DEV bool shadow_visible(const DeviceScene& sc, const SceneRecs& recs, const Stack& stack, V3 p0, V3 p1) {
    V3 d = p1 - p0;
    float len = length(d);
    d = d / len;
    float tfar = len * (1.0f - 0.00001f);
    Hit hit; hit.t = tfar; hit.u = 0.0f; hit.v = 0.0f; hit.prim = -1;
    V3 inv_d = mk3(div_rn(1.0f, d.x), div_rn(1.0f, d.y), div_rn(1.0f, d.z));
    float te;
    if (!slab(mk3(sc.root_min[0], sc.root_min[1], sc.root_min[2]), mk3(sc.root_max[0], sc.root_max[1], sc.root_max[2]), p0, inv_d, kEps, tfar, &te))
        return false;
    return !traverse<true>(recs, Stack::kBvh4 ? sc.root4 : sc.root, mk3(sc.root_min[0], sc.root_min[1], sc.root_min[2]), mk3(sc.root_max[0], sc.root_max[1], sc.root_max[2]),
                           p0, d, kEps, tfar, hit, stack);
}
template <class Stack>
RL_DEV bool trace_closest(const DeviceScene& sc, const SceneRecs& recs, const Stack& stack, V3 o, V3 d, Hit& hit) {
    hit.t = kF32Max; hit.u = 0.0f; hit.v = 0.0f; hit.prim = -1;
    traverse<false>(recs, sc.root, mk3(sc.root_min[0], sc.root_min[1], sc.root_min[2]), mk3(sc.root_max[0], sc.root_max[1], sc.root_max[2]),
                    o, d, kEps, kF32Max, hit, stack);
    return hit.prim >= 0;
}
template <class Stack>
RL_DEV bool trace_none(const DeviceScene& sc, const SceneRecs& recs, const Stack& stack, V3 o, V3 d) {
    Hit hit; hit.t = kF32Max; hit.u = 0.0f; hit.v = 0.0f; hit.prim = -1;
    return !traverse<true>(recs, sc.root, mk3(sc.root_min[0], sc.root_min[1], sc.root_min[2]), mk3(sc.root_max[0], sc.root_max[1], sc.root_max[2]),
                           o, d, kEps, kF32Max, hit, stack);
}
template <class PS, class Stack>
RL_DEV void shadow_slot(const DeviceScene& sc, const SceneRecs& recs, const Stack& stack, PS& ps) {
    if (shadow_visible(sc, recs, stack, load3(ps, F_OX), load3(ps, F_SX))) storec(ps, F_LR, loadc(ps, F_LR) + loadc(ps, F_CR));
}

template <int MAT, bool MEDIUM, int LIGHTS = LIGHTS_ANY, bool DRAWS_ONLY = false, class SMP = Rng, class PS>
RL_DEV void shade_slot(const RenderConst& rc, const DeviceScene& sc, PS& ps, unsigned flags,
                       unsigned& n_vertices, unsigned& n_draws, unsigned& n_shadow, unsigned& n_ext) {
    n_ext += 1;
    const unsigned prev = (flags >> ST_PREV_SHIFT) & 3u;
    const unsigned depth = PU(U_DEPTH);
    const int prim = (int)PU(U_PRIM);
    const bool primary = prev == PREV_SENSOR;
    const V3 ro = primary ? mk3(sc.camera.position[0], sc.camera.position[1], sc.camera.position[2]) : load3(ps, F_OX);
    const V3 rd = load3(ps, F_DX);
    const float t_hit = PF(F_T);
    Col w_edge = (primary || DRAWS_ONLY) ? cone() : loadc(ps, F_WR);
    const float rr = (primary || DRAWS_ONLY) ? 1.0f : PF(F_RR);
    const float pdf_edge = (primary || DRAWS_ONLY) ? 1.0f : PF(F_PDF);
    Col beta = (primary || DRAWS_ONLY) ? cone() : loadc(ps, F_BR);
    Col L = (primary || DRAWS_ONLY) ? czero() : loadc(ps, F_LR);
    bool zeroed = (flags & ST_ZEROED) != 0u;
    const bool hit = prim >= 0;
    bool is_volume = false;
    V3 vpos = mk3(0.0f, 0.0f, 0.0f);
    if (MEDIUM) {
        MediumSample ms = medium_sample(sc.medium, hit ? t_hit : kF32Max, PF(F_XI));
        w_edge = w_edge * ms.w;
        is_volume = !hit || !ms.exited;
        if (is_volume) vpos = ro + rd * ms.t;
    }
    bool ended = false;
    unsigned new_flags = ST_REGEN;
    unsigned smp_bits = 0u;
    if (!MEDIUM && !hit) {
        ended = true;
        if constexpr (!DRAWS_ONLY) {
        Col contrib = (w_edge * rr) * (LIGHTS != LIGHTS_AREA_ONLY && sc.env_emitter >= 0 ? env_eval(sc, rd) : czero());
        const bool add_contrib = rc.has_min ? (depth - 1u) >= rc.min_depth : true;
        if (prev == PREV_SENSOR) {
            if (!is_zero(contrib) && add_contrib) L = L + contrib;
        } else if (!zeroed) {
            if (rc.strategy == RL_STRATEGY_EMITTER) contrib = czero();
            Col term = czero();
            if (!is_zero(contrib) && add_contrib) {
                float wmis = 1.0f;
                if (rc.strategy == RL_STRATEGY_ALL && (flags & ST_PDF_SA)) {
                    float p2 = (LIGHTS != LIGHTS_AREA_ONLY && (prev == PREV_SURFACE || prev == PREV_VOLUME)) ? env_direct_pdf(sc, rd) : 0.0f;
                    float total = (0.0f + pdf_edge) + p2;
                    wmis = div_rn(pdf_edge, total);
                }
                term = contrib * wmis;
            }
            L = L + beta * term;
        }
        storec(ps, F_LR, L);
        }
    }
    if (!ended) {
        const Col W = w_edge * rr;
        SurfacePoint sp;
        const Material* mat = nullptr;
        MeshRecord mr;
        if (!is_volume) {
            sp = fill_intersection(sc, prim, PF(F_U), PF(F_V), ro, rd, t_hit);
            mr = sc.meshes[sp.mesh];
            mat = &sc.materials[mr.material];
        }
        if constexpr (!DRAWS_ONLY) {
        Col emit = czero();
        if (!is_volume && (mr.flags & MESH_IS_LIGHT) && dot(sp.n_s, -rd) >= 0.0f) emit = mesh_emit<LIGHTS>(sc, mr, sp.has_uv, sp.uv);
        Col contrib = W * emit;
        const unsigned cur = depth - 1u;
        const bool add_contrib = rc.has_min ? cur >= rc.min_depth : true;
        if (prev == PREV_SENSOR) {
            if (!is_zero(contrib) && add_contrib) L = L + contrib;
        } else if (!zeroed) {
// ... 138 lines not shown
```

### rustlight_amd/csrc/kernels/wavefront.h

```cpp
#pragma once
#include <stddef.h>
#include <stdint.h>
#include <string>

struct rl_context;
struct rl_scene;
void rl_set_error(const std::string& s);

extern "C" {
int rl_debug_numerics(int device, size_t n, const float* a, const float* b, float* out8);
enum rl_math_fn { RL_MATH_SINF = 0, RL_MATH_COSF = 1, RL_MATH_EXPF = 2, RL_MATH_LOGF = 3, RL_MATH_POWF = 4, RL_MATH_ACOSF = 5, RL_MATH_ATAN2F = 6, RL_MATH_ASINF = 7,
                  RL_MATH_SQRT_RN = 8, RL_MATH_DIV_RN = 9, RL_MATH_MUL_ADD = 10 , RL_MATH_COUNT = 11 };
enum rl_math_where { RL_MATH_ON_DEVICE = 0, RL_MATH_ON_HOST = 1 };
int rl_debug_math_sweep(int device, int where, int fn, uint32_t first_bits, uint32_t stride, uint32_t period, size_t n, const float* b, size_t n_b, int swap, float* out);
int rl_debug_trace_batch_fast(rl_context* ctx, size_t n, const float* origins, const float* directions, float* t_out, int32_t* mesh_out, int32_t* tri_out, int32_t* steps_out);
int rl_debug_trace_batch_two_level(rl_context* ctx, size_t n, const float* origins, const float* directions, float* t_inout, float* u_out, float* v_out,
                                   int32_t* mesh_out, int32_t* tri_out, int32_t* steps_out, int any_hit);
int rl_debug_check_two_level(const rl_scene* scene, uint64_t* out6);
int rl_debug_rng_advance(int device, size_t n, const uint64_t* states_in, const uint32_t* counts, uint64_t* states_out);
int rl_debug_stratified_draws(int device, size_t n_pixels, const uint64_t* pixel_seeds, uint32_t spp, int seed_variant, size_t n_calls, const int32_t* pattern, float* out);
int rl_debug_trivial_pixels(const rl_scene* scene, int has_max_depth, uint32_t max_depth, uint8_t* out);
int rl_debug_bvh_sizes(const rl_context* ctx, uint64_t* n_ref_nodes, uint64_t* n_prims, uint32_t* stack_depth, int* lds_scene);
int rl_debug_bvh(const rl_scene* scene, uint64_t* n_nodes, uint64_t* n_prims, float* boxes, uint64_t* info, uint64_t* count,
                 int32_t* prim_mesh, int32_t* prim_tri);
int rl_debug_emitters_cdf(const rl_scene* scene, uint64_t* n_entries, float* cdf);
int rl_debug_ats(const rl_scene* scene, uint64_t* n_nodes, float* nodes16, uint64_t* n_lights, int32_t* light_emitter, int32_t* light_prim);
int rl_debug_camera_ray(const rl_scene* scene, float px, float py, float* origin, float* direction);
}
```

### rustlight_amd/csrc/kernels/wavefront.hip

```cpp
#include <hip/hip_runtime.h>

#include <algorithm>
#include <chrono>
#include <cmath>
#include <cstdio>
#include <cstring>
#include <memory>
#include <string>
#include <thread>
#include <vector>

#include "common.hip.h"
#include "rngjump.h"
#include "../host/hip_buffer.h"
#include "../host/photontree.h"
#include "phototree.h"
#include "../host/scene.h"
#include "wavefront.h"
#include "knobs.h"
#include "light.hip.h"

namespace rl {

__global__ void k_seed_pixels(RenderConst rc) {
    unsigned j = blockIdx.x * blockDim.x + threadIdx.x;
    if (j >= rc.n_owned) return;
    unsigned b = rc.owned_blocks[j];
    unsigned bx, by, bw, bh;
    block_geometry(rc, b, &bx, &by, &bw, &bh);
    Rng rng = rng_seed(rc.block_seeds[b], rc.seed_variant);
    unsigned base = rc.block_item_base[j];
    for (unsigned iy = 0; iy < bh; iy++)
        for (unsigned ix = 0; ix < bw; ix++) {
            unsigned k = base + iy * bw + ix;
            rc.item_seed[k] = rng_next_u64(rng);
            rc.item_pixel[k] = (by + iy) * rc.W + (bx + ix);
        }
}

__global__ void k_chunk_pixels(RenderConst rc) {
    unsigned j = blockIdx.x * blockDim.x + threadIdx.x;
    if (j >= rc.n_owned) return;
    unsigned bx, by, bw, bh;
    block_geometry(rc, rc.owned_blocks[j], &bx, &by, &bw, &bh);
    const unsigned c_end = min(rc.cursor_end, bw * bh), base = rc.block_item_base[j];
    for (unsigned c = rc.cursor_begin; c < c_end; c++) rc.item_pixel[base + (c - rc.cursor_begin)] = (by + c / bw) * rc.W + (bx + c % bw);
}

__global__ void k_init(RenderConst rc, Pool pool) {
    unsigned slot = blockIdx.x * blockDim.x + threadIdx.x;
    if (slot >= pool.P) return;
    PoolState ps{pool, slot};
    PU(U_ITEM) = slot;
    PU(U_CURSOR) = 0u;
    PU(U_SAMPLE) = 0u;
    PU(U_DEPTH) = 0u;
    PU(U_PRIM) = 0xffffffffu;
    PU(U_FLAGS) = slot < rc.n_items ? (ST_REGEN | ST_FRESH) : ST_FINISHED;
    storec(ps, F_AR, czero());
    storec(ps, F_LR, czero());
}

__global__ void __launch_bounds__(256) k_raygen(RenderConst rc, DeviceScene sc, Pool pool) {
    unsigned n_samples = 0, n_draws = 0;
    for (unsigned slot = blockIdx.x * blockDim.x + threadIdx.x; slot < pool.P; slot += gridDim.x * blockDim.x) {
        PoolState ps{pool, slot};
        raygen_slot<true>(rc, sc, ps, n_samples, n_draws);
    }
    { const int which[2] = {STAT_SAMPLES, STAT_DRAWS}; const unsigned vals[2] = {n_samples, n_draws}; block_stats<2>(rc.partials, which, vals); }
}

__global__ void __launch_bounds__(256) k_fold_samples(RenderConst rc) {
    const unsigned n_pix = rc.n_items / rc.split;
    const unsigned p = blockIdx.x * blockDim.x + threadIdx.x;
    if (p >= n_pix) return;
    Col acc = czero();
    for (unsigned s = 0; s < rc.spp; s++) {
        const float* src = rc.sample_buf + 3 * ((size_t)s * n_pix + p);
        acc = acc + mkc(src[0], src[1], src[2]);
    }
    const Col px = scale_unguarded(acc, rc.inv_spp);
    const size_t pix = rc.item_pixel[p];
    rc.out[3 * pix] = px.r; rc.out[3 * pix + 1] = px.g; rc.out[3 * pix + 2] = px.b;
}

#ifdef RL_TRAV_STATS
__device__ unsigned long long g_trav_stats[8];
#endif
template <bool LDS_SCENE, bool SHADOW>
RL_DEV void trace_kernel_body(const DeviceScene& sc, const Pool& pool, const StackConf& stc) {
    extern __shared__ __attribute__((aligned(16))) float4 smem[];
    float4* after_scene = LDS_SCENE ? smem + lds_scene_float4s(sc.n_nodes, sc.n_prims) : smem;
    unsigned* list = reinterpret_cast<unsigned*>(after_scene);
    unsigned slot = blockIdx.x * blockDim.x + threadIdx.x;
    const TravStackT<LDS_SCENE> stack = make_stack<LDS_SCENE>(stc, list + 272, slot);
    const unsigned flags = slot < pool.P ? pool.u[(size_t)U_FLAGS * pool.P + slot] : 0u;
    const unsigned n_live = block_compact((flags & (SHADOW ? ST_SHADOW : ST_RAY)) != 0u, slot, list);
    if (n_live == 0u) return;
    SceneRecs recs;
    if (LDS_SCENE) {
        stage_scene_lds(sc, smem, smem + lds_nodes_float4s(sc.n_nodes));
        recs.nodes = smem; recs.tris = smem + lds_nodes_float4s(sc.n_nodes);
    } else {
        recs.nodes = streamed_nodes<TravStackT<false>>(sc);
        recs.tris = reinterpret_cast<const float4*>(sc.tris);
    }
#ifdef RL_TRAV_STATS
    int dbg[2] = {-1, 0};
    if (threadIdx.x < n_live) {
        PoolState ps{pool, list[threadIdx.x]};
        if (SHADOW) shadow_slot(sc, recs, stack, ps);
        else extend_slot(sc, recs, stack, ps, dbg);
    }
    if (!SHADOW) {
        int mx = dbg[0];
        for (int off = 32; off > 0; off >>= 1) mx = max(mx, __shfl_xor(mx, off, 64));
        if (dbg[0] >= 0) { atomicAdd(&g_trav_stats[0], 1ull); atomicAdd(&g_trav_stats[1], (unsigned long long)dbg[0]); atomicAdd(&g_trav_stats[2], (unsigned long long)dbg[1]); if (dbg[0] == 0) atomicAdd(&g_trav_stats[5], 1ull); }
        if ((threadIdx.x & 63u) == 0u && mx >= 0) { atomicAdd(&g_trav_stats[3], 64ull * (unsigned long long)mx); atomicAdd(&g_trav_stats[4], 1ull); }
    }
#else
    if (threadIdx.x < n_live) {
        PoolState ps{pool, list[threadIdx.x]};
        if (SHADOW) shadow_slot(sc, recs, stack, ps);
        else extend_slot(sc, recs, stack, ps);
    }
#endif
}

template <bool LDS_SCENE>
__global__ void __launch_bounds__(256) k_extend(RenderConst rc, DeviceScene sc, Pool pool, StackConf stc) { trace_kernel_body<LDS_SCENE, false>(sc, pool, stc); }
template <bool LDS_SCENE>
__global__ void __launch_bounds__(256) k_shadow(RenderConst rc, DeviceScene sc, Pool pool, StackConf stc) { trace_kernel_body<LDS_SCENE, true>(sc, pool, stc); }

__global__ void __launch_bounds__(256) k_trace_batch(DeviceScene sc, StackConf stc, unsigned n, const float* o, const float* d, float* t_out, float* u_out,
                                                     float* v_out, int* mesh_out, int* tri_out) {
    extern __shared__ __attribute__((aligned(16))) float4 smem[];
    SceneRecs recs;
    recs.nodes = streamed_nodes<TravStackT<false>>(sc);
    recs.tris = reinterpret_cast<const float4*>(sc.tris);
    unsigned i = blockIdx.x * blockDim.x + threadIdx.x;
    const TravStack stack = make_stack(stc, reinterpret_cast<unsigned*>(smem), i);
    if (i >= n) return;
    V3 ro = mk3(o[3 * i], o[3 * i + 1], o[3 * i + 2]), rd = mk3(d[3 * i], d[3 * i + 1], d[3 * i + 2]);
    Hit hit;
    trace_closest(sc, recs, stack, ro, rd, hit);
    t_out[i] = hit.t; u_out[i] = hit.u; v_out[i] = hit.v;
    if (hit.prim >= 0) { mesh_out[i] = sc.tris[hit.prim].mesh; tri_out[i] = sc.tris[hit.prim].tri; }
    else { mesh_out[i] = -1; tri_out[i] = -1; }
}

__global__ void __launch_bounds__(256) k_trace_batch_two_level(DeviceScene sc, StackConf stc, unsigned n, const float* o, const float* d, float* t_out, float* u_out,
                                                               float* v_out, int* mesh_out, int* tri_out, int* steps_out, int any_hit) {
    extern __shared__ __attribute__((aligned(16))) float4 smem[];
    SceneRecs recs;
    recs.nodes = reinterpret_cast<const float4*>(sc.nodes2);
    recs.tris = reinterpret_cast<const float4*>(sc.tris);
    unsigned i = blockIdx.x * blockDim.x + threadIdx.x;
    const TravStack2 stack(make_stack(stc, reinterpret_cast<unsigned*>(smem), i));
    if (i >= n) return;
    V3 ro = mk3(o[3 * i], o[3 * i + 1], o[3 * i + 2]), rd = mk3(d[3 * i], d[3 * i + 1], d[3 * i + 2]);
    Hit hit; hit.t = kF32Max; hit.u = 0.0f; hit.v = 0.0f; hit.prim = -1;
    if (any_hit) {
        hit.t = t_out[i];
        const bool f = traverse<true>(recs, sc.root, mk3(sc.root_min[0], sc.root_min[1], sc.root_min[2]), mk3(sc.root_max[0], sc.root_max[1], sc.root_max[2]), ro, rd, kEps, hit.t, hit, stack);
        t_out[i] = f ? 1.0f : 0.0f; steps_out[i] = hit.steps;
        return;
    }
    trace_closest(sc, recs, stack, ro, rd, hit);
    t_out[i] = hit.t; u_out[i] = hit.u; v_out[i] = hit.v; steps_out[i] = hit.steps;
    if (hit.prim >= 0) { mesh_out[i] = sc.tris[hit.prim].mesh; tri_out[i] = sc.tris[hit.prim].tri; }
    else { mesh_out[i] = -1; tri_out[i] = -1; }
}

__global__ void __launch_bounds__(256) k_visible_batch(DeviceScene sc, StackConf stc, unsigned n, const float* p0a, const float* p1a, unsigned char* out) {
    extern __shared__ __attribute__((aligned(16))) float4 smem[];
    SceneRecs recs;
    recs.nodes = streamed_nodes<TravStackT<false>>(sc);
    recs.tris = reinterpret_cast<const float4*>(sc.tris);
    unsigned i = blockIdx.x * blockDim.x + threadIdx.x;
    const TravStack stack = make_stack(stc, reinterpret_cast<unsigned*>(smem), i);
    if (i >= n) return;
    V3 p0 = mk3(p0a[3 * i], p0a[3 * i + 1], p0a[3 * i + 2]), p1 = mk3(p1a[3 * i], p1a[3 * i + 1], p1a[3 * i + 2]);
    out[i] = shadow_visible(sc, recs, stack, p0, p1) ? 1 : 0;
}

__global__ void k_numerics_probe(unsigned n, const float* a, const float* b, float* out_div, float* out_sqrt, float* out_mad, float* out_sin,
                                 float* out_cos, float* out_exp, float* out_log, float* out_pow, float* out_acos, float* out_atan2) {
    unsigned i = blockIdx.x * blockDim.x + threadIdx.x;
    if (i >= n) return;
    out_div[i] = div_rn(a[i], b[i]);
    out_sqrt[i] = sqrt_rn(fabsf(a[i]));
    out_mad[i] = a[i] * b[i] + a[i];
    out_sin[i] = dm::sinf_det(a[i]);
    out_cos[i] = dm::cosf_det(a[i]);
    out_exp[i] = dm::expf_det(a[i]);
    out_log[i] = dm::logf_det(fabsf(a[i]));
    out_pow[i] = dm::powf_det(fabsf(a[i]), b[i]);
    out_acos[i] = dm::acosf_det(a[i] * 0.15f);
    out_atan2[i] = dm::atan2f_det(a[i], b[i]);
}

__global__ void k_math_sweep(int fn, int swap, unsigned first_bits, unsigned stride, unsigned period, unsigned n, const float* b, float b_const, float* out) {
    unsigned i = blockIdx.x * blockDim.x + threadIdx.x;
    if (i >= n) return;
    const float g = __uint_as_float(first_bits + (period ? i % period : i) * stride);
    const float c = b ? b[i] : b_const;
    const float x = swap ? c : g, y = swap ? g : c;
    float r;
    switch (fn) {
        case RL_MATH_SINF: r = dm::sinf_det(x); break;
        case RL_MATH_COSF: r = dm::cosf_det(x); break;
        case RL_MATH_EXPF: r = dm::expf_det(x); break;
        case RL_MATH_LOGF: r = dm::logf_det(x); break;
        case RL_MATH_POWF: r = dm::powf_det(x, y); break;
        case RL_MATH_ACOSF: r = dm::acosf_det(x); break;
        case RL_MATH_ATAN2F: r = dm::atan2f_det(x, y); break;
        case RL_MATH_ASINF: r = dm::asinf_det(x); break;
        case RL_MATH_SQRT_RN: r = sqrt_rn(x); break;
        case RL_MATH_DIV_RN: r = div_rn(x, y); break;
        default: r = x * y + x; break;
    }
    out[i] = r;
}

}

using namespace rl;

static thread_local std::string g_last_error;
void rl_set_error(const std::string& s) { g_last_error = s; }
extern "C" const char* rl_last_error(void) { return g_last_error.c_str(); }

struct rl_context {
    int device = 0;
    hipStream_t stream = nullptr;
    DeviceScene ds{};
    std::vector<HipBuffer<unsigned char>> allocs;
    uint32_t width = 0, height = 0;
    bool single_bsdf = true;
    int bsdf_type = 0;
    bool lds_scene = false;
    bool area_lights_only = false;
    bool has_directional = false;
    size_t scene_lds_bytes = 0;
    size_t lds_limit = 64 * 1024;
    HipBuffer<float> pool_f; HipBuffer<unsigned> pool_u; HipBuffer<unsigned long long> pool_q;
    HipBuffer<unsigned> d_owned, d_item_base;
    HipBuffer<unsigned long long> d_block_seeds, d_item_seed;
    HipBuffer<unsigned> d_item_pixel;
    HipBuffer<float> d_out;
    HipBuffer<Counters> d_counters;
    HipBuffer<Counters, Mem::Pinned> h_counters;
    HipBuffer<unsigned long long> d_partials;
    HipBuffer<int> d_overflow;
    HipBuffer<int> d_overflow2;
    HipBuffer<float> d_sample_buf;
    HipBuffer<unsigned long long> d_sample_states;
    HipBuffer<unsigned long long> d_chain_states;
    HipBuffer<unsigned> d_trk_off;
    HipBuffer<ulonglong2> d_trk_st;
    HipBuffer<unsigned> d_trivial;
    uint64_t trivial_key = ~0ull;
    HipBuffer<unsigned long long> d_spec_stats;
    std::vector<hipEvent_t> events;
    static constexpr int kEvalStreams = 4;
    hipStream_t stream2 = nullptr; hipStream_t eval_streams[kEvalStreams] = {};
    HipBuffer<unsigned> d_queue;
    hipEvent_t ev_chain_done = nullptr;
    HipBuffer<unsigned, Mem::Mapped> h_flags;
    HipBuffer<unsigned, Mem::Pinned> h_list;
    unsigned queue_seq = 0;
    BvhBuild bvh_dump;
    Knobs knobs;
    LightConst light_cam{};
    std::vector<RectLight> rect_lights;
    int rect_lights_rc = RL_OK;
    std::string rect_lights_err;
};

template <typename T>
static int upload(rl_context* ctx, const std::vector<T>& v, const T** out) {
    *out = nullptr;
    ctx->allocs.emplace_back();
    HipBuffer<unsigned char>& b = ctx->allocs.back();
    int rcode;
    if ((rcode = b.ensure(std::max<size_t>(v.size(), 1) * sizeof(T))) != RL_OK) return rcode;
    if (!v.empty()) HIP_OK(hipMemcpy(b.get(), v.data(), v.size() * sizeof(T), hipMemcpyHostToDevice));
    *out = reinterpret_cast<const T*>(b.get());
    return RL_OK;
}

static int ensure_two_level(rl_context* ctx) {
    if (ctx->ds.nodes2) return RL_OK;
    std::vector<BvhNode2> n2;
    two_level_nodes(ctx->bvh_dump, &n2);
    return upload(ctx, n2, &ctx->ds.nodes2);
}

extern "C" int rl_device_count(int* count) {
    if (!count) return RL_ERR_INVALID_ARGUMENT;
    int n = 0;
    if (hipGetDeviceCount(&n) != hipSuccess || n <= 0) { *count = 0; return RL_ERR_NO_DEVICE; }
    *count = n;
    return RL_OK;
}

extern "C" int rl_context_create(const rl_scene* scene, int device, rl_context** out) {
    if (!scene || !out) return RL_ERR_INVALID_ARGUMENT;
    if (!scene->has_camera) return RL_ERR_INVALID_ARGUMENT;
    if (!scene->emitters_built) return RL_ERR_NOT_BUILT;
    int n_dev = 0;
    hipError_t e = hipGetDeviceCount(&n_dev);
    if (e != hipSuccess || n_dev <= 0) {
        rl_set_error("no HIP device available (hipGetDeviceCount); the MI355X path has no CPU fallback");
        return RL_ERR_NO_DEVICE;
    }
    if (device < 0 || device >= n_dev) { rl_set_error("device ordinal out of range"); return RL_ERR_NO_DEVICE; }
    HIP_OK(hipSetDevice(device));
    rl_context* ctx = new rl_context();
    ctx->device = device;
    ctx->width = scene->width; ctx->height = scene->height;
    ctx->knobs.from_environment();
    int rc = RL_OK;
    do {
        {
            int prio_least = 0, prio_greatest = 0;
            if (hipDeviceGetStreamPriorityRange(&prio_least, &prio_greatest) != hipSuccess) { (void)hipGetLastError(); prio_least = prio_greatest = 0; }
            if (hipStreamCreateWithPriority(&ctx->stream, hipStreamNonBlocking, prio_greatest) != hipSuccess) { rl_set_error("hipStreamCreate failed"); rc = RL_ERR_HIP; break; }
            if (hipStreamCreateWithPriority(&ctx->stream2, hipStreamNonBlocking, prio_least) != hipSuccess) { (void)hipGetLastError(); ctx->stream2 = nullptr; }
            if (ctx->stream2 && hipEventCreateWithFlags(&ctx->ev_chain_done, hipEventDisableTiming) != hipSuccess) { (void)hipGetLastError(); hipStreamDestroy(ctx->stream2); ctx->stream2 = nullptr; }
            if (ctx->stream2) {
                ctx->eval_streams[0] = ctx->stream2;
                for (int k = 1; k < rl_context::kEvalStreams; k++)
                    if (hipStreamCreateWithPriority(&ctx->eval_streams[k], hipStreamNonBlocking, prio_least) != hipSuccess) { (void)hipGetLastError(); ctx->eval_streams[k] = ctx->stream2; }
            }
        }
        BvhBuild& bvh = ctx->bvh_dump;
        build_bvh(*scene, &bvh);
        FlatScene flat;
        flatten_scene(*scene, &flat);
        DeviceScene& ds = ctx->ds;
        if ((rc = upload(ctx, bvh.nodes, &ds.nodes)) != RL_OK) break;
        if ((rc = upload(ctx, bvh.tris, &ds.tris)) != RL_OK) break;
        for (int i = 0; i < 3; i++) { ds.root_min[i] = bvh.root_min[i]; ds.root_max[i] = bvh.root_max[i]; }
        ds.root = bvh.root;
        ds.n_nodes = (uint32_t)bvh.nodes.size();
        ds.n_prims = (uint32_t)bvh.tris.size();
        ds.stack_depth = bvh.stack_depth;
        ds.nodes4 = nullptr; ds.root4 = RL_CHILD_NONE; ds.stack_depth4 = 0;
        ds.nodes_t = nullptr; ds.root_t = RL_CHILD_NONE;
        ds.nodes2 = nullptr;
        if ((rc = upload(ctx, flat.tri_indices, &ds.tri_indices)) != RL_OK) break;
        if ((rc = upload(ctx, flat.positions, &ds.positions)) != RL_OK) break;
        if ((rc = upload(ctx, flat.normals, &ds.normals)) != RL_OK) break;
        if ((rc = upload(ctx, flat.uvs, &ds.uvs)) != RL_OK) break;
        for (MeshRecord& mr : flat.meshes) mr.ats_base = 0xffffffffu;
        std::vector<int32_t> ats_light_mesh;
        if (scene->ats_root >= 0) {
            for (size_t e = 0; e < scene->emitters.size(); e++) flat.meshes[scene->emitters[e].mesh].ats_base = scene->ats_emitter_base[e];
            for (int32_t e : scene->ats_light_emitter) ats_light_mesh.push_back(scene->emitters[e].mesh);
        }
        if ((rc = upload(ctx, flat.meshes, &ds.meshes)) != RL_OK) break;
        ds.ats_root = scene->ats_root;
        if ((rc = upload(ctx, scene->ats_nodes, &ds.ats_nodes)) != RL_OK) break;
        if ((rc = upload(ctx, ats_light_mesh, &ds.ats_light_mesh)) != RL_OK) break;
        if ((rc = upload(ctx, scene->ats_light_prim, &ds.ats_light_prim)) != RL_OK) break;
        if ((rc = upload(ctx, scene->ats_leaf_of, &ds.ats_leaf_of)) != RL_OK) break;
        if ((rc = upload(ctx, flat.materials, &ds.materials)) != RL_OK) break;
        if ((rc = upload(ctx, flat.bitmaps, &ds.bitmaps)) != RL_OK) break;
        if ((rc = upload(ctx, flat.bitmap_texels, &ds.bitmap_texels)) != RL_OK) break;
        if ((rc = upload(ctx, scene->emitters, &ds.emitters)) != RL_OK) break;
        if ((rc = upload(ctx, scene->emitters_cdf, &ds.emitters_cdf)) != RL_OK) break;
        ds.n_emitters = (uint32_t)scene->emitters.size();
        ds.env_emitter = -1;
        for (size_t e = 0; e < scene->emitters.size(); e++)
            if (scene->emitters[e].kind == EMITTER_ENV) {
                ds.env_emitter = (int32_t)e;
                for (int k = 0; k < 3; k++) ds.env_color[k] = scene->emitters[e].c[k];
                ds.env_pdf = (1.0f / (3.14159265358979323846f * 4.0f)) * (scene->emitters_cdf[e + 1] - scene->emitters_cdf[e]);
                ds.env_sel_pdf = scene->emitters_cdf[e + 1] - scene->emitters_cdf[e];
            }
        ds.env_w = ds.env_h = 0;
        if (ds.env_emitter >= 0 && scene->env_map.w) {
            ds.env_w = scene->env_map.w; ds.env_h = scene->env_map.h;
            ds.env_marg_func_int = scene->env_marg_func_int;
            if ((rc = upload(ctx, scene->env_map.rgb, &ds.env_texels)) != RL_OK) break;
            if ((rc = upload(ctx, scene->env_cond_cdf, &ds.env_cond_cdf)) != RL_OK) break;
            if ((rc = upload(ctx, scene->env_cond_func, &ds.env_cond_func)) != RL_OK) break;
            if ((rc = upload(ctx, scene->env_marg_cdf, &ds.env_marg_cdf)) != RL_OK) break;
        }
        if (ds.env_emitter >= 0 && scene->medium.enabled) { rl_set_error("an environment emitter cannot be combined with a medium (paths/edge.rs:94)"); rc = RL_ERR_UNSUPPORTED; break; }
        if ((rc = upload(ctx, flat.mesh_cdf, &ds.mesh_cdf)) != RL_OK) break;
        ds.n_meshes = (uint32_t)flat.meshes.size();
        scene->sample_to_camera.to_cols(ds.camera.sample_to_camera);
        scene->to_world.to_cols(ds.camera.to_world);
        ds.camera.position[0] = scene->cam_pos.x; ds.camera.position[1] = scene->cam_pos.y; ds.camera.position[2] = scene->cam_pos.z;
        ds.camera.width = scene->width; ds.camera.height = scene->height;
        {
            scene->camera_to_sample.to_cols(ctx->light_cam.camera_to_sample);
            scene->to_local.to_cols(ctx->light_cam.to_local);
            const Vec3 p0 = scene->sample_to_camera.xform_point({0.0f, 0.0f, 0.0f}), p1 = scene->sample_to_camera.xform_point({1.0f, 1.0f, 0.0f});
            const float zmin = std::fmin(p0.z, p1.z), zmax = std::fmax(p0.z, p1.z);
            ctx->light_cam.rect_min[0] = std::fmin(p0.x, p1.x) / zmin; ctx->light_cam.rect_min[1] = std::fmin(p0.y, p1.y) / zmin;
            ctx->light_cam.rect_max[0] = std::fmax(p0.x, p1.x) / zmax; ctx->light_cam.rect_max[1] = std::fmax(p0.y, p1.y) / zmax;
        }
        ds.medium = scene->medium;
        {
            const char* why = "";
            if ((ctx->rect_lights_rc = build_rect_lights(*scene, &ctx->rect_lights, &why)) != RL_OK) ctx->rect_lights_err = why;
        }
        ctx->area_lights_only = scene->ats_root < 0 && !ctx->knobs.has(K_GENERIC_LIGHTS);
        for (const EmitterRecord& e : scene->emitters) if (e.kind != EMITTER_MESH) ctx->area_lights_only = false;
        for (const EmitterRecord& e : scene->emitters) if (e.kind == EMITTER_DIRECTIONAL) ctx->has_directional = true;
        for (const HostMesh& hm : scene->meshes) if (hm.is_light && hm.emission_type != RL_EMISSION_COLOR) ctx->area_lights_only = false;
        ctx->single_bsdf = true;
        ctx->bsdf_type = flat.materials.empty() ? 0 : flat.materials[0].type;
        for (const Material& m : flat.materials) if (m.type != ctx->bsdf_type) ctx->single_bsdf = false;
        ctx->scene_lds_bytes = (size_t)16 * lds_scene_float4s(ds.n_nodes, ds.n_prims);
        ctx->lds_scene = ctx->scene_lds_bytes <= 48 * 1024 && ds.stack_depth <= (uint32_t)kLdsStackLevels;
        {
            int lds_limit = 64 * 1024;
            if (hipDeviceGetAttribute(&lds_limit, hipDeviceAttributeMaxSharedMemoryPerBlock, device) != hipSuccess) { (void)hipGetLastError(); lds_limit = 64 * 1024; }
            ctx->lds_limit = (size_t)std::max(lds_limit, 16 * 1024);
            const size_t worst = ctx->scene_lds_bytes + std::max<size_t>(272 * sizeof(unsigned), kFusedColdBytes) + (size_t)2 * kLdsStackLevels * 256 * sizeof(int);
            if (worst > (size_t)lds_limit) ctx->lds_scene = false;
        }
        if (ctx->knobs.has(K_FORCE_STREAMING)) ctx->lds_scene = false;
        if (!ctx->lds_scene) {
            Bvh4Build b4;
            build_bvh4(bvh, &b4);
            if ((rc = upload(ctx, b4.nodes, &ds.nodes4)) != RL_OK) break;
            ds.root4 = b4.root; ds.stack_depth4 = b4.stack_depth;
            std::vector<BvhNode> blocks;
            int32_t root_t = RL_CHILD_NONE;
            treelet_blocks(bvh, &blocks, &root_t);
            if ((rc = upload(ctx, blocks, &ds.nodes_t)) != RL_OK) break;
            ds.root_t = root_t;
        }
        if (ctx->d_counters.ensure(1) != RL_OK) { rl_set_error("hipMalloc counters"); rc = RL_ERR_HIP; break; }
        if (ctx->h_counters.ensure(1) != RL_OK) { rl_set_error("hipHostMalloc counters"); rc = RL_ERR_HIP; break; }
    } while (0);
    if (rc != RL_OK) { rl_context_destroy(ctx); return rc; }
    *out = ctx;
    return RL_OK;
}

extern "C" void rl_context_destroy(rl_context* ctx) {
    if (!ctx) return;
    hipSetDevice(ctx->device);
    for (hipEvent_t ev : ctx->events) hipEventDestroy(ev);
    if (ctx->ev_chain_done) hipEventDestroy(ctx->ev_chain_done);
    for (int k = 1; k < rl_context::kEvalStreams; k++) if (ctx->eval_streams[k] && ctx->eval_streams[k] != ctx->stream2) hipStreamDestroy(ctx->eval_streams[k]);
    if (ctx->stream2) hipStreamDestroy(ctx->stream2);
    if (ctx->stream) hipStreamDestroy(ctx->stream);
    delete ctx;
}

#ifndef RL_LDS_LEVELS_STREAMING
#define RL_LDS_LEVELS_STREAMING 6
#endif
static constexpr int kLdsStackLevelsStreaming = RL_LDS_LEVELS_STREAMING;
static int lds_levels_of(const rl_context* ctx) { return std::min<int>((int)ctx->ds.stack_depth, ctx->lds_scene ? kLdsStackLevels : kLdsStackLevelsStreaming); }
static size_t traversal_lds_bytes(const rl_context* ctx, bool lds_scene, unsigned block, bool with_list, int lds_levels = -1) {
    size_t stack = (size_t)2 * (lds_levels >= 0 ? lds_levels : lds_levels_of(ctx)) * block * sizeof(int);
    return (lds_scene ? ctx->scene_lds_bytes : 0) + (with_list ? 272 * sizeof(unsigned) : 0) + stack;
}
static int stack_conf(rl_context* ctx, size_t n_threads, StackConf* out, bool second = false, int lds_levels = -1) {
    HipBuffer<int>& d_overflow = second ? ctx->d_overflow2 : ctx->d_overflow;
    out->lds_levels = lds_levels >= 0 ? std::min(lds_levels, lds_levels_of(ctx)) : lds_levels_of(ctx);
    out->pre_group = 0;
    out->overflow = nullptr;
    out->overflow_stride = n_threads;
    int extra = (int)std::max(ctx->ds.stack_depth, ctx->ds.stack_depth4) - out->lds_levels;
    if (extra > 0) {
        const int rcode = d_overflow.ensure((size_t)2 * extra * n_threads);
        if (rcode != RL_OK) return rcode;
        out->overflow = d_overflow.get();
    }
    return RL_OK;
}

struct BlockRect { unsigned x, y, w, h; };
static BlockRect block_rect(size_t b, size_t nby, uint32_t W, uint32_t H) {
    const unsigned x = (unsigned)(b / nby) * 16u, y = (unsigned)(b % nby) * 16u;
    return {x, y, std::min(16u, W - x), std::min(16u, H - y)};
}

struct TrivialInput { uint32_t W, H; bool medium, empty; float root_min[3], root_max[3]; CameraRecord camera; };
static TrivialInput trivial_input(const rl_context* ctx) {
    TrivialInput in{};
    in.W = ctx->width; in.H = ctx->height; in.medium = ctx->ds.medium.enabled != 0; in.empty = ctx->ds.root == RL_CHILD_NONE || ctx->ds.n_prims == 0;
    for (int k = 0; k < 3; k++) { in.root_min[k] = ctx->ds.root_min[k]; in.root_max[k] = ctx->ds.root_max[k]; }
    in.camera = ctx->ds.camera;
    return in;
}
static void trivial_pixel_masks(const TrivialInput& ti, const rl_path_params* params, const std::vector<unsigned>& owned, size_t nby, bool no_shortcut, std::vector<unsigned>* out) {
    const uint32_t W = ti.W, H = ti.H;
    out->assign(owned.size() * 8, 0u);
    const bool expand = !params->has_max_depth || 1u < params->max_depth;
    auto all_of_block = [&](size_t j, unsigned npx) { for (unsigned c = 0; c < npx; c++) (*out)[j * 8 + (c >> 5)] |= 1u << (c & 31u); };
    if (!expand) {
        for (size_t j = 0; j < owned.size(); j++) { const BlockRect r = block_rect(owned[j], nby, W, H); all_of_block(j, r.w * r.h); }
        return;
    }
    if (ti.medium || no_shortcut) return;
    const bool empty = ti.empty;
    double lo[3], hi[3];
    for (int k = 0; k < 3; k++) {
        lo[k] = ti.root_min[k]; hi[k] = ti.root_max[k];
        if (!empty && !(std::isfinite(lo[k]) && std::isfinite(hi[k]) && lo[k] <= hi[k])) return;
        const double grow = 1e-3 * (hi[k] - lo[k]) + 1e-4 * std::max(1.0, std::max(std::fabs(lo[k]), std::fabs(hi[k])));
        lo[k] -= grow; hi[k] += grow;
    }
    const float* m = ti.camera.sample_to_camera; const float* tw = ti.camera.to_world;
    const double cam[3] = {ti.camera.position[0], ti.camera.position[1], ti.camera.position[2]};
    auto ray_dir = [&](double u, double v, double* d) -> bool {
        const double sx = u / (double)W, sy = v / (double)H;
        const double hx = m[0] * sx + m[4] * sy + m[12], hy = m[1] * sx + m[5] * sy + m[13], hz = m[2] * sx + m[6] * sy + m[14], hw = m[3] * sx + m[7] * sy + m[15];
        if (!(std::fabs(hw) > 1e-12) || !std::isfinite(hx + hy + hz + hw)) return false;
        const double nx = hx / hw, ny = hy / hw, nz = hz / hw;
        d[0] = tw[0] * nx + tw[4] * ny + tw[8] * nz; d[1] = tw[1] * nx + tw[5] * ny + tw[9] * nz; d[2] = tw[2] * nx + tw[6] * ny + tw[10] * nz;
        d[3] = hw;
        const double len = std::sqrt(d[0] * d[0] + d[1] * d[1] + d[2] * d[2]);
        if (!(len > 1e-30) || !std::isfinite(len)) return false;
        d[0] /= len; d[1] /= len; d[2] /= len;
        return true;
    };
    auto misses = [&](double u0, double v0, double u1, double v1) -> bool {
        if (empty) return true;
        double d[4][4];
        const double us[4] = {u0, u1, u1, u0}, vs[4] = {v0, v0, v1, v1};
        for (int k = 0; k < 4; k++) if (!ray_dir(us[k], vs[k], d[k])) return false;
        for (int k = 1; k < 4; k++) if ((d[k][3] > 0) != (d[0][3] > 0)) return false;
        for (int k = 0; k < 4; k++) {
            const double* a = d[k]; const double* b = d[(k + 1) & 3]; const double* o = d[(k + 2) & 3];
            double n[3] = {a[1] * b[2] - a[2] * b[1], a[2] * b[0] - a[0] * b[2], a[0] * b[1] - a[1] * b[0]};
            const double nl = std::sqrt(n[0] * n[0] + n[1] * n[1] + n[2] * n[2]);
            if (!(nl > 1e-14)) return false;
            double inside = (n[0] * o[0] + n[1] * o[1] + n[2] * o[2]) / nl;
            if (!(std::fabs(inside) > 1e-9)) return false;
            const double sgn = inside > 0 ? 1.0 : -1.0;
            bool all_out = true;
            for (int cbit = 0; cbit < 8 && all_out; cbit++) {
                const double p[3] = {((cbit & 1) ? hi[0] : lo[0]) - cam[0], ((cbit & 2) ? hi[1] : lo[1]) - cam[1], ((cbit & 4) ? hi[2] : lo[2]) - cam[2]};
                const double pl = std::sqrt(p[0] * p[0] + p[1] * p[1] + p[2] * p[2]);
                const double s = sgn * (n[0] * p[0] + n[1] * p[1] + n[2] * p[2]) / nl;
                if (!(s < -1e-7 * pl - 1e-12)) all_out = false;
            }
            if (all_out) return true;
        }
        return false;
    };
    for (size_t j = 0; j < owned.size(); j++) {
        const BlockRect r = block_rect(owned[j], nby, W, H);
        const unsigned bx = r.x, by = r.y, bw = r.w, bh = r.h;
        if (misses(bx - 0.25, by - 0.25, bx + bw + 0.25, by + bh + 0.25)) { all_of_block(j, bw * bh); continue; }
        for (unsigned c = 0; c < bw * bh; c++) {
            const double x = bx + c % bw, y = by + c / bw;
            if (misses(x - 0.25, y - 0.25, x + 1.25, y + 1.25)) (*out)[j * 8 + (c >> 5)] |= 1u << (c & 31u);
        }
    }
}

extern "C" int rl_debug_trivial_pixels(const rl_scene* scene, int has_max_depth, uint32_t max_depth, uint8_t* out) {
    if (!scene || !out || !scene->has_camera) return RL_ERR_INVALID_ARGUMENT;
    BvhBuild bvh;
    build_bvh(*scene, &bvh);
    TrivialInput ti{};
    ti.W = scene->width; ti.H = scene->height; ti.medium = scene->medium.enabled != 0; ti.empty = bvh.root == RL_CHILD_NONE || bvh.tris.empty();
    for (int k = 0; k < 3; k++) { ti.root_min[k] = bvh.root_min[k]; ti.root_max[k] = bvh.root_max[k]; }
    scene->sample_to_camera.to_cols(ti.camera.sample_to_camera);
    scene->to_world.to_cols(ti.camera.to_world);
    ti.camera.position[0] = scene->cam_pos.x; ti.camera.position[1] = scene->cam_pos.y; ti.camera.position[2] = scene->cam_pos.z;
    ti.camera.width = scene->width; ti.camera.height = scene->height;
    rl_path_params pp{};
    pp.has_max_depth = has_max_depth; pp.max_depth = max_depth;
    const size_t nbx = (ti.W + 15) / 16, nby = (ti.H + 15) / 16;
    std::vector<unsigned> owned(nbx * nby), masks;
    for (size_t b = 0; b < owned.size(); b++) owned[b] = (unsigned)b;
    trivial_pixel_masks(ti, &pp, owned, nby, false, &masks);
    std::memset(out, 0, (size_t)ti.W * ti.H);
    for (size_t b = 0; b < owned.size(); b++) {
        const BlockRect r = block_rect(b, nby, ti.W, ti.H);
        for (unsigned c = 0; c < r.w * r.h; c++) if ((masks[b * 8 + (c >> 5)] >> (c & 31u)) & 1u) out[(size_t)(r.y + c / r.w) * ti.W + r.x + c % r.w] = 1;
    }
    return RL_OK;
}

static int check_frame(const rl_context* ctx, uint32_t spp, const uint64_t* block_seeds, size_t n_blocks, const float* out_rgb) {
    if (!ctx || !block_seeds || !out_rgb) return RL_ERR_INVALID_ARGUMENT;
    if (n_blocks != (size_t)((ctx->width + 15) / 16) * ((ctx->height + 15) / 16)) { rl_set_error("n_blocks does not match the image size"); return RL_ERR_INVALID_ARGUMENT; }
    if (spp == 0) { rl_set_error("spp must be > 0 (assert_ne!(scene.nb_samples, 0), mod.rs:410)"); return RL_ERR_INVALID_ARGUMENT; }
    return RL_OK;
}
template <typename Params>
static int check_frame(const rl_context* ctx, const Params* params, const uint64_t* block_seeds, size_t n_blocks, const float* out_rgb) {
    return params ? check_frame(ctx, params->spp, block_seeds, n_blocks, out_rgb) : RL_ERR_INVALID_ARGUMENT;
}
static int check_streams(int32_t stream_mode, uint32_t spp, uint32_t numerics, uint32_t shard_index, uint32_t shard_count) {
    if (stream_mode < RL_STREAM_REFERENCE_ORDER || stream_mode > RL_STREAM_STRATIFIED) { rl_set_error("stream_mode must be 0 (reference order), 1 (per sample) or 2 (stratified)"); return RL_ERR_INVALID_ARGUMENT; }
    if (stream_mode == RL_STREAM_STRATIFIED && spp > (1u << 30)) { rl_set_error("the stratified sampler takes at most 2^30 spp"); return RL_ERR_INVALID_ARGUMENT; }
    if (numerics > RL_NUMERICS_FAST) { rl_set_error("numerics must be 0 (exact) or 1 (fast)"); return RL_ERR_INVALID_ARGUMENT; }
    if (shard_index >= (shard_count ? shard_count : 1)) return RL_ERR_INVALID_ARGUMENT;
    return RL_OK;
}

namespace {

struct RenderFrame {
    rl_context* const ctx;
    const uint64_t* const block_seeds;
    const size_t n_blocks;
    float* const out_rgb;
    const int out_is_device;
    const hipStream_t st;
    rl_render_stats* const stats;
    const Knobs knobs;
    const uint32_t W, H;
    const size_t nby;
    const uint32_t shard_count;
    const std::chrono::steady_clock::time_point t_start;
    const bool timing;
    int cus = 256;
    std::vector<unsigned> owned, item_base;
    unsigned n_pixels = 0;
    float* d_out = nullptr;
    size_t n_rows = 0;
    unsigned long long totals[STAT_COUNT] = {};

    RenderFrame(rl_context* c, const uint64_t* seeds, size_t nb, float* out, int out_dev, void* stream_arg, rl_render_stats* s, uint32_t shard_index, uint32_t n_shards)
        : ctx(c), block_seeds(seeds), n_blocks(nb), out_rgb(out), out_is_device(out_dev), st(stream_arg ? (hipStream_t)stream_arg : c->stream), stats(s),
          knobs(c->knobs), W(c->width), H(c->height), nby((c->height + 15) / 16), shard_count(n_shards ? n_shards : 1), t_start(std::chrono::steady_clock::now()),
          timing(s != nullptr && !knobs.has(K_NO_EVENTS)) {
        for (size_t b = 0; b < n_blocks; b++) {
            if (b % shard_count != shard_index) continue;
            const BlockRect r = block_rect(b, nby, W, H);
            owned.push_back((unsigned)b);
            item_base.push_back(n_pixels);
            n_pixels += r.w * r.h;
        }
        hipDeviceGetAttribute(&cus, hipDeviceAttributeMultiprocessorCount, ctx->device);
    }

    size_t max_state_bytes() const { return knobs.has(K_STATE_BUDGET_MB) ? std::max<size_t>(1, (size_t)knobs.i(K_STATE_BUDGET_MB, 0)) << 20 : (size_t)24 << 30; }

    int alloc_tables() {
        int rcode;
        if ((rcode = ctx->d_owned.ensure(owned.size())) != RL_OK || (rcode = ctx->d_item_base.ensure(owned.size())) != RL_OK ||
            (rcode = ctx->d_block_seeds.ensure(n_blocks)) != RL_OK) return rcode;
        return RL_OK;
    }
    int alloc_output(size_t rows) {
        d_out = out_rgb;
        if (!out_is_device) {
            const int rcode = ctx->d_out.ensure((size_t)3 * W * H);
            if (rcode != RL_OK) return rcode;
            d_out = ctx->d_out.get();
        }
        n_rows = rows;
        return ctx->d_partials.ensure(n_rows * STAT_COUNT);
    }
    int upload(bool with_item_base, bool zero_image) {
        HIP_OK(hipMemcpyAsync(ctx->d_owned.get(), owned.data(), owned.size() * sizeof(unsigned), hipMemcpyHostToDevice, st));
        if (with_item_base) HIP_OK(hipMemcpyAsync(ctx->d_item_base.get(), item_base.data(), item_base.size() * sizeof(unsigned), hipMemcpyHostToDevice, st));
        HIP_OK(hipMemcpyAsync(ctx->d_block_seeds.get(), block_seeds, n_blocks * sizeof(uint64_t), hipMemcpyHostToDevice, st));
        if (zero_image) HIP_OK(hipMemsetAsync(d_out, 0, (size_t)3 * W * H * sizeof(float), st));
        return RL_OK;
    }
    int zero_rows() {
        HIP_OK(hipMemsetAsync(ctx->d_partials.get(), 0, n_rows * STAT_COUNT * sizeof(unsigned long long), st));
        return RL_OK;
    }
    RenderConst render_const(uint32_t spp, int32_t stream_mode, int32_t seed_variant) const {
        RenderConst rc{};
        rc.spp = spp;
        rc.stream_mode = stream_mode; rc.seed_variant = seed_variant;
        rc.inv_spp = 1.0f / (float)spp;
        rc.W = W; rc.H = H; rc.nby = (unsigned)nby;
        rc.owned_blocks = ctx->d_owned.get(); rc.block_item_base = ctx->d_item_base.get(); rc.n_owned = (unsigned)owned.size();
        rc.block_seeds = ctx->d_block_seeds.get();
        rc.item_seed = ctx->d_item_seed.get(); rc.item_pixel = ctx->d_item_pixel.get();
        rc.out = d_out;
        rc.counters = ctx->d_counters.get();
        rc.partials = ctx->d_partials.get();
        return rc;
    }
    int grow_events(size_t n) {
        if (timing) while (ctx->events.size() < n) { hipEvent_t ev; HIP_OK(hipEventCreate(&ev)); ctx->events.push_back(ev); }
        return RL_OK;
    }
    int download() {
        if (!out_is_device) HIP_OK(hipMemcpyAsync(out_rgb, d_out, (size_t)3 * W * H * sizeof(float), hipMemcpyDeviceToHost, st));
        std::vector<unsigned long long> partials(n_rows * STAT_COUNT);
        HIP_OK(hipMemcpyAsync(partials.data(), ctx->d_partials.get(), partials.size() * sizeof(unsigned long long), hipMemcpyDeviceToHost, st));
        HIP_OK(hipStreamSynchronize(st));
        HIP_OK(hipGetLastError());
        for (size_t r = 0; r < n_rows; r++) for (int k = 0; k < STAT_COUNT; k++) totals[k] += partials[r * STAT_COUNT + k];
        if (stats) {
            std::memset(stats, 0, sizeof(*stats));
            stats->camera_samples = totals[STAT_SAMPLES]; stats->vertices = totals[STAT_VERTICES]; stats->extension_rays = totals[STAT_EXT_RAYS];
            stats->shadow_rays = totals[STAT_SHADOW_RAYS]; stats->rng_draws = totals[STAT_DRAWS];
            stats->render_ms = std::chrono::duration<double, std::milli>(std::chrono::steady_clock::now() - t_start).count();
        }
        return RL_OK;
    }
};

struct LaneRun {
    std::vector<unsigned long long> words;
// ... 438 lines not shown
                float t = 0.0f;
                if (hipEventElapsedTime(&t, ctx->events[2 * s], ctx->events[2 * s + 1]) == hipSuccess) raygen += t;
                hipEvent_t end = s + 1 < params->spp ? ctx->events[2 * (s + 1)] : ctx->events[2 * (size_t)params->spp];
                if (hipEventElapsedTime(&t, ctx->events[2 * s + 1], end) == hipSuccess) gather += t;
            }
            stats->ms_raygen = raygen; stats->ms_other = gather;
            (void)hipGetLastError();
        }
    }
    return RL_OK;
}

#include "gather_render.hip.h"

namespace {
constexpr size_t kMaxBatch = 0x7fffff00u;
}
extern "C" int rl_trace_batch(rl_context* ctx, size_t n, const float* origins, const float* directions, float* t_out, float* u_out,
                              float* v_out, int32_t* mesh_out, int32_t* tri_out) {
    if (!ctx || (n && (!origins || !directions || !t_out || !u_out || !v_out || !mesh_out || !tri_out))) return RL_ERR_INVALID_ARGUMENT;
    if (n == 0) return RL_OK;
    if (n > kMaxBatch) { rl_set_error("batch too large"); return RL_ERR_INVALID_ARGUMENT; }
    HIP_OK(hipSetDevice(ctx->device));
    HipBuffer<float> b_o, b_d, b_t, b_u, b_v; HipBuffer<int> b_m, b_tr;
    int rcode;
    if ((rcode = b_o.ensure(3 * n)) != RL_OK || (rcode = b_d.ensure(3 * n)) != RL_OK || (rcode = b_t.ensure(n)) != RL_OK || (rcode = b_u.ensure(n)) != RL_OK ||
        (rcode = b_v.ensure(n)) != RL_OK || (rcode = b_m.ensure(n)) != RL_OK || (rcode = b_tr.ensure(n)) != RL_OK) return rcode;
    float *d_o = b_o.get(), *d_d = b_d.get(), *d_t = b_t.get(), *d_u = b_u.get(), *d_v = b_v.get();
    int *d_m = b_m.get(), *d_tr = b_tr.get();
    HIP_OK(hipMemcpy(d_o, origins, 3 * n * 4, hipMemcpyHostToDevice));
    HIP_OK(hipMemcpy(d_d, directions, 3 * n * 4, hipMemcpyHostToDevice));
    size_t lds = traversal_lds_bytes(ctx, false, 256, false);
    StackConf stc;
    if ((rcode = stack_conf(ctx, (n + 255) / 256 * 256, &stc)) != RL_OK) return rcode;
    hipLaunchKernelGGL(k_trace_batch, dim3((unsigned)((n + 255) / 256)), dim3(256), lds, ctx->stream, ctx->ds, stc, (unsigned)n, d_o, d_d, d_t, d_u, d_v, d_m, d_tr);
    HIP_OK(hipGetLastError());
    HIP_OK(hipStreamSynchronize(ctx->stream));
    HIP_OK(hipMemcpy(t_out, d_t, n * 4, hipMemcpyDeviceToHost)); HIP_OK(hipMemcpy(u_out, d_u, n * 4, hipMemcpyDeviceToHost));
    HIP_OK(hipMemcpy(v_out, d_v, n * 4, hipMemcpyDeviceToHost)); HIP_OK(hipMemcpy(mesh_out, d_m, n * 4, hipMemcpyDeviceToHost));
    HIP_OK(hipMemcpy(tri_out, d_tr, n * 4, hipMemcpyDeviceToHost));
    return RL_OK;
}

extern "C" int rl_visible_batch(rl_context* ctx, size_t n, const float* p0, const float* p1, uint8_t* visible_out) {
    if (!ctx || (n && (!p0 || !p1 || !visible_out))) return RL_ERR_INVALID_ARGUMENT;
    if (n == 0) return RL_OK;
    if (n > kMaxBatch) { rl_set_error("batch too large"); return RL_ERR_INVALID_ARGUMENT; }
    HIP_OK(hipSetDevice(ctx->device));
    HipBuffer<float> b_a, b_b; HipBuffer<unsigned char> b_o;
    int rcode;
    if ((rcode = b_a.ensure(3 * n)) != RL_OK || (rcode = b_b.ensure(3 * n)) != RL_OK || (rcode = b_o.ensure(n)) != RL_OK) return rcode;
    float *d_a = b_a.get(), *d_b = b_b.get(); unsigned char* d_o = b_o.get();
    HIP_OK(hipMemcpy(d_a, p0, 3 * n * 4, hipMemcpyHostToDevice));
    HIP_OK(hipMemcpy(d_b, p1, 3 * n * 4, hipMemcpyHostToDevice));
    size_t lds = traversal_lds_bytes(ctx, false, 256, false);
    StackConf stc;
    if ((rcode = stack_conf(ctx, (n + 255) / 256 * 256, &stc)) != RL_OK) return rcode;
    hipLaunchKernelGGL(k_visible_batch, dim3((unsigned)((n + 255) / 256)), dim3(256), lds, ctx->stream, ctx->ds, stc, (unsigned)n, d_a, d_b, d_o);
    HIP_OK(hipGetLastError());
    HIP_OK(hipStreamSynchronize(ctx->stream));
    HIP_OK(hipMemcpy(visible_out, d_o, n, hipMemcpyDeviceToHost));
    return RL_OK;
}

extern "C" int rl_debug_numerics(int device, size_t n, const float* a, const float* b, float* out8) {
    int n_dev = 0;
    if (hipGetDeviceCount(&n_dev) != hipSuccess || n_dev <= 0) return RL_ERR_NO_DEVICE;
    if (n > kMaxBatch / 16) return RL_ERR_INVALID_ARGUMENT;
    HIP_OK(hipSetDevice(device));
    HipBuffer<float> b_a, b_b, b_out;
    int rcode;
    if ((rcode = b_a.ensure(n)) != RL_OK || (rcode = b_b.ensure(n)) != RL_OK || (rcode = b_out.ensure(10 * n)) != RL_OK) return rcode;
    float *d_a = b_a.get(), *d_b = b_b.get(), *d_out = b_out.get();
    HIP_OK(hipMemcpy(d_a, a, n * 4, hipMemcpyHostToDevice)); HIP_OK(hipMemcpy(d_b, b, n * 4, hipMemcpyHostToDevice));
    hipLaunchKernelGGL(k_numerics_probe, dim3((unsigned)((n + 255) / 256)), dim3(256), 0, 0, (unsigned)n, d_a, d_b, d_out, d_out + n, d_out + 2 * n,
                       d_out + 3 * n, d_out + 4 * n, d_out + 5 * n, d_out + 6 * n, d_out + 7 * n, d_out + 8 * n, d_out + 9 * n);
    HIP_OK(hipGetLastError());
    HIP_OK(hipDeviceSynchronize());
    HIP_OK(hipMemcpy(out8, d_out, 10 * n * 4, hipMemcpyDeviceToHost));
    return RL_OK;
}

extern "C" int rl_debug_math_sweep(int device, int where, int fn, uint32_t first_bits, uint32_t stride, uint32_t period, size_t n, const float* b, size_t n_b,
                                   int swap, float* out) {
    if (fn < 0 || fn >= RL_MATH_COUNT || !out || n == 0 || (n_b != 0 && !b) || (n_b != 0 && n_b != 1 && n_b != n)) return RL_ERR_INVALID_ARGUMENT;
    if (n > kMaxBatch) { rl_set_error("batch too large"); return RL_ERR_INVALID_ARGUMENT; }
    if (where == RL_MATH_ON_HOST) return host_math_sweep(fn, first_bits, stride, period, n, b, n_b, swap, out);
    if (where != RL_MATH_ON_DEVICE) return RL_ERR_INVALID_ARGUMENT;
    int n_dev = 0;
    if (hipGetDeviceCount(&n_dev) != hipSuccess || n_dev <= 0) return RL_ERR_NO_DEVICE;
    HIP_OK(hipSetDevice(device));
    HipBuffer<float> b_b, b_out;
    int rcode;
    if ((rcode = b_out.ensure(n)) != RL_OK || (n_b == n && n > 1 && (rcode = b_b.ensure(n)) != RL_OK)) return rcode;
    const float* d_b = nullptr;
    if (n_b == n && n > 1) { HIP_OK(hipMemcpy(b_b.get(), b, n * 4, hipMemcpyHostToDevice)); d_b = b_b.get(); }
    hipLaunchKernelGGL(k_math_sweep, dim3((unsigned)((n + 255) / 256)), dim3(256), 0, 0, fn, swap, (unsigned)first_bits, (unsigned)stride, (unsigned)period, (unsigned)n,
                       d_b, n_b ? b[0] : 0.0f, b_out.get());
    HIP_OK(hipGetLastError());
    HIP_OK(hipDeviceSynchronize());
    HIP_OK(hipMemcpy(out, b_out.get(), n * 4, hipMemcpyDeviceToHost));
    return RL_OK;
}

extern "C" int rl_debug_trace_batch_fast(rl_context* ctx, size_t n, const float* origins, const float* directions, float* t_out, int32_t* mesh_out, int32_t* tri_out, int32_t* steps_out) {
    if (!ctx || !n || !origins || !directions || !t_out || !mesh_out || !tri_out || !steps_out) return RL_ERR_INVALID_ARGUMENT;
    if (!ctx->ds.nodes4) { rl_set_error("the scene is staged in LDS: no BVH4"); return RL_ERR_UNSUPPORTED; }
    if (n > kMaxBatch) { rl_set_error("batch too large"); return RL_ERR_INVALID_ARGUMENT; }
    HIP_OK(hipSetDevice(ctx->device));
    HipBuffer<float> b_o, b_d, b_t; HipBuffer<int> b_m, b_tr, b_s;
    int rcode;
    if ((rcode = b_o.ensure(3 * n)) != RL_OK || (rcode = b_d.ensure(3 * n)) != RL_OK || (rcode = b_t.ensure(n)) != RL_OK || (rcode = b_m.ensure(n)) != RL_OK ||
        (rcode = b_tr.ensure(n)) != RL_OK || (rcode = b_s.ensure(n)) != RL_OK) return rcode;
    HIP_OK(hipMemcpy(b_o.get(), origins, 3 * n * 4, hipMemcpyHostToDevice));
    HIP_OK(hipMemcpy(b_d.get(), directions, 3 * n * 4, hipMemcpyHostToDevice));
    StackConf stc;
    if ((rcode = stack_conf(ctx, (n + 255) / 256 * 256, &stc)) != RL_OK) return rcode;
    launch_trace_batch_fast(dim3((unsigned)((n + 255) / 256)), dim3(256), traversal_lds_bytes(ctx, false, 256, false), ctx->stream, ctx->ds, stc, (unsigned)n, b_o.get(), b_d.get(),
                            b_t.get(), b_m.get(), b_tr.get(), b_s.get());
    HIP_OK(hipGetLastError());
    HIP_OK(hipStreamSynchronize(ctx->stream));
    HIP_OK(hipMemcpy(t_out, b_t.get(), n * 4, hipMemcpyDeviceToHost)); HIP_OK(hipMemcpy(mesh_out, b_m.get(), n * 4, hipMemcpyDeviceToHost));
    HIP_OK(hipMemcpy(tri_out, b_tr.get(), n * 4, hipMemcpyDeviceToHost)); HIP_OK(hipMemcpy(steps_out, b_s.get(), n * 4, hipMemcpyDeviceToHost));
    return RL_OK;
}

extern "C" int rl_debug_trace_batch_two_level(rl_context* ctx, size_t n, const float* origins, const float* directions, float* t_inout, float* u_out, float* v_out,
                                              int32_t* mesh_out, int32_t* tri_out, int32_t* steps_out, int any_hit) {
    if (!ctx || !n || !origins || !directions || !t_inout || !u_out || !v_out || !mesh_out || !tri_out || !steps_out) return RL_ERR_INVALID_ARGUMENT;
    if (n > kMaxBatch) { rl_set_error("batch too large"); return RL_ERR_INVALID_ARGUMENT; }
    HIP_OK(hipSetDevice(ctx->device));
    { const int r2 = ensure_two_level(ctx); if (r2 != RL_OK) return r2; }
    HipBuffer<float> b_o, b_d, b_t, b_u, b_v; HipBuffer<int> b_m, b_tr, b_s;
    int rcode;
    if ((rcode = b_o.ensure(3 * n)) != RL_OK || (rcode = b_d.ensure(3 * n)) != RL_OK || (rcode = b_t.ensure(n)) != RL_OK || (rcode = b_u.ensure(n)) != RL_OK ||
        (rcode = b_v.ensure(n)) != RL_OK || (rcode = b_m.ensure(n)) != RL_OK || (rcode = b_tr.ensure(n)) != RL_OK || (rcode = b_s.ensure(n)) != RL_OK) return rcode;
    HIP_OK(hipMemcpy(b_o.get(), origins, 3 * n * 4, hipMemcpyHostToDevice));
    HIP_OK(hipMemcpy(b_d.get(), directions, 3 * n * 4, hipMemcpyHostToDevice));
    HIP_OK(hipMemcpy(b_t.get(), t_inout, n * 4, hipMemcpyHostToDevice));
    StackConf stc;
    if ((rcode = stack_conf(ctx, (n + 255) / 256 * 256, &stc)) != RL_OK) return rcode;
    hipLaunchKernelGGL(k_trace_batch_two_level, dim3((unsigned)((n + 255) / 256)), dim3(256), traversal_lds_bytes(ctx, false, 256, false), ctx->stream, ctx->ds, stc, (unsigned)n,
                       b_o.get(), b_d.get(), b_t.get(), b_u.get(), b_v.get(), b_m.get(), b_tr.get(), b_s.get(), any_hit);
    HIP_OK(hipGetLastError());
    HIP_OK(hipStreamSynchronize(ctx->stream));
    HIP_OK(hipMemcpy(t_inout, b_t.get(), n * 4, hipMemcpyDeviceToHost)); HIP_OK(hipMemcpy(steps_out, b_s.get(), n * 4, hipMemcpyDeviceToHost));
    if (!any_hit) {
        HIP_OK(hipMemcpy(u_out, b_u.get(), n * 4, hipMemcpyDeviceToHost)); HIP_OK(hipMemcpy(v_out, b_v.get(), n * 4, hipMemcpyDeviceToHost));
        HIP_OK(hipMemcpy(mesh_out, b_m.get(), n * 4, hipMemcpyDeviceToHost)); HIP_OK(hipMemcpy(tri_out, b_tr.get(), n * 4, hipMemcpyDeviceToHost));
    }
    return RL_OK;
}

extern "C" int rl_debug_bvh_sizes(const rl_context* ctx, uint64_t* n_ref_nodes, uint64_t* n_prims, uint32_t* stack_depth, int* lds_scene) {
    if (!ctx) return RL_ERR_INVALID_ARGUMENT;
    *n_ref_nodes = ctx->bvh_dump.ref_info.size(); *n_prims = ctx->bvh_dump.ref_prim_mesh.size();
    *stack_depth = ctx->bvh_dump.stack_depth; *lds_scene = ctx->lds_scene ? 1 : 0;
    return RL_OK;
}

extern "C" const char* rl_build_info(void) { return "rustlight_amd wavefront path tracer; kernels: gfx950 (hipcc, -ffp-contract=off)"; }
```

Baseline: 5235.

## Split the last heavy pixel blocks across several lanes to shorten the fused-kernel tail

For large diffuse area-light scenes rendered with the fused per-sample kernel, the planner picks the last up to 512 non-trivial pixel blocks and gives each of their pixels several lanes (default 4) instead of one. Their per-sample radiance goes to a sample buffer and is folded by an extra k_fold_samples launch. The goal is to cut the load-imbalance tail, where the last long-running workgroups leave most CUs idle at the end of the launch. In exchange it adds more items, a buffer write per sample, an extra kernel launch, a new template variant, and host-side trivial-block analysis. Stage-timer instrumentation for per-workgroup lifetimes is also added.

After: 5494 (median of 6 runs). 5.0% higher.

```diff
diff --git a/rustlight_amd/api.py b/rustlight_amd/api.py
--- a/rustlight_amd/api.py
+++ b/rustlight_amd/api.py
@@ -428,6 +428,13 @@
     def set_option(self, name: str, value=None):
         _check(lib().rl_context_set_option(self.h, name.lower().encode(), None if value is None else str(value).encode()))
 
+    def sample_buf_bytes(self) -> int:
+        n = C.c_uint64(0)
+        fn = lib().rl_debug_sample_buf_bytes
+        fn.argtypes = [C.c_void_p, C.POINTER(C.c_uint64)]
+        _check(fn(self.h, C.byref(n)))
+        return int(n.value)
+
     def get_option(self, name: str):
         v = lib().rl_context_get_option(self.h, name.lower().encode())
         return None if v is None else v.decode()
diff --git a/rustlight_amd/csrc/kernels/fused.hip.h b/rustlight_amd/csrc/kernels/fused.hip.h
--- a/rustlight_amd/csrc/kernels/fused.hip.h
+++ b/rustlight_amd/csrc/kernels/fused.hip.h
@@ -13,20 +13,25 @@
 
 #ifdef RL_STAGE_TIMERS
 __device__ unsigned long long g_stage_timers[32];
+static constexpr unsigned kFusedWgSlots = 1u << 15;
+static __device__ unsigned long long g_fused_wgs[2 * kFusedWgSlots];
 #endif
 template <int MAT, bool MEDIUM, bool LDS_SCENE, int LIGHTS, int NUM, bool QUEUE = false>
 __global__ void __launch_bounds__(256, LDS_SCENE ? RL_FUSED_WAVES : RL_FUSED_WAVES_STREAMING) k_path_fused(RenderConst rc_arg, DeviceScene sc_arg, StackConf stc) {
     using SMP = Rng;
+#define RL_FUSED_BODY_TAIL ((NUM & 2) != 0 && !QUEUE && LDS_SCENE && !MEDIUM)
 #include "fused_body.inc.h"
+#undef RL_FUSED_BODY_TAIL
 }
 
 
 template <bool LDS_SCENE>
 static void launch_fused_impl(int mat, bool medium, bool area_only, dim3 grid, dim3 block, size_t lds_bytes, hipStream_t st, const RenderConst& rc, const DeviceScene& ds, const StackConf& stc) {
-    with_bsdf(mat, [&](auto M) { with_flag(medium, [&](auto MED) { with_flag(area_only, [&](auto AREA) {
+    with_bsdf(mat, [&](auto M) { with_flag(medium, [&](auto MED) { with_flag(area_only, [&](auto AREA) { with_flag(rc.tail_lanes != 0u, [&](auto TAIL) {
         constexpr int MAT = decltype(M)::value, LIGHTS = decltype(AREA)::value ? LIGHTS_AREA_ONLY : LIGHTS_ANY;
-        hipLaunchKernelGGL((k_path_fused<MAT, decltype(MED)::value, LDS_SCENE, LIGHTS, RL_NUMERICS_ID, RL_FUSED_QUEUE != 0>), grid, block, lds_bytes, st, rc, ds, stc);
-    }); }); });
+        constexpr int NUM = RL_NUMERICS_ID + ((decltype(TAIL)::value && LDS_SCENE && !decltype(MED)::value && RL_FUSED_QUEUE == 0) ? 2 : 0);
+        hipLaunchKernelGGL((k_path_fused<MAT, decltype(MED)::value, LDS_SCENE, LIGHTS, NUM, RL_FUSED_QUEUE != 0>), grid, block, lds_bytes, st, rc, ds, stc);
+    }); }); }); });
 }
 template <bool LDS_SCENE>
 static void dump_stage_timers_impl() {
@@ -44,6 +49,35 @@
                                  100.0 * h[21] / pr, 100.0 * h[22] / pr, 100.0 * h[23] / pr, 100.0 * h[24] / pr);
     }
     std::memset(h, 0, sizeof(h)); hipMemcpyToSymbol(HIP_SYMBOL(g_stage_timers), h, sizeof(h));
+    {
+        std::vector<unsigned long long> w(2 * (size_t)kFusedWgSlots);
+        hipMemcpyFromSymbol(w.data(), HIP_SYMBOL(g_fused_wgs), w.size() * 8);
+        std::vector<std::pair<double, double>> wg;
+        unsigned long long t_first = ~0ull;
+        for (size_t i = 0; i < kFusedWgSlots; i++) if (w[2 * i + 1]) t_first = std::min(t_first, w[2 * i]);
+        for (size_t i = 0; i < kFusedWgSlots; i++) if (w[2 * i + 1]) wg.push_back({(w[2 * i] - t_first) * 1e-5, (w[2 * i + 1] - t_first) * 1e-5});
+        int dev = 0, cus = 256;
+        (void)hipGetDevice(&dev); (void)hipDeviceGetAttribute(&cus, hipDeviceAttributeMultiprocessorCount, dev);
+        const double slots = (double)cus * (LDS_SCENE ? RL_FUSED_WAVES : RL_FUSED_WAVES_STREAMING);
+        if (wg.size() >= 16) {
+            auto pct = [](std::vector<double> v, double q) { std::sort(v.begin(), v.end()); return v[std::min(v.size() - 1, (size_t)(q * (double)v.size()))]; };
+            std::vector<double> life, heavy;
+            double span = 0.0, busy_total = 0.0, last_heavy_start = 0.0;
+            for (const auto& g : wg) { life.push_back(g.second - g.first); span = std::max(span, g.second); busy_total += g.second - g.first; }
+            const double cut = 0.25 * pct(life, 0.9);
+            for (const auto& g : wg) if (g.second - g.first >= cut) { heavy.push_back(g.second - g.first); last_heavy_start = std::max(last_heavy_start, g.first); }
+            const double L = pct(heavy, 0.5), L90 = pct(heavy, 0.9), win0 = std::max(0.0, span - 1.5 * L);
+            double busy_win = 0.0;
+            for (const auto& g : wg) busy_win += std::max(0.0, g.second - std::max(g.first, win0));
+            std::fprintf(stderr, "[tail] %zu workgroups (%zu heavy) on %.0f slots, launch %.3f ms; heavy lifetime median %.3f ms, p90 %.3f ms, max %.3f ms; last heavy workgroup starts at %.3f ms\n",
+                         wg.size(), heavy.size(), slots, span, L, L90, pct(heavy, 1.0), last_heavy_start);
+            std::fprintf(stderr, "[tail] busy slots over the last 1.5 L (from %.3f ms, every L / 8):", win0);
+            for (int k = 0; k <= 12; k++) { const double t = win0 + (span - win0) * k / 12.0; unsigned n = 0; for (const auto& g : wg) if (g.first <= t && t < g.second) n++; std::fprintf(stderr, " %u", n); }
+            std::fprintf(stderr, "\n[tail] idle slot-time in that window %.2f slot-ms = %.2f %% of slots x launch; over the whole launch %.2f %%\n",
+                         slots * (span - win0) - busy_win, 100.0 * (slots * (span - win0) - busy_win) / (slots * span), 100.0 * (slots * span - busy_total) / (slots * span));
+        }
+        std::fill(w.begin(), w.end(), 0ull); hipMemcpyToSymbol(HIP_SYMBOL(g_fused_wgs), w.data(), w.size() * 8);
+    }
 #endif
 }
 
diff --git a/rustlight_amd/csrc/kernels/fused_body.inc.h b/rustlight_amd/csrc/kernels/fused_body.inc.h
--- a/rustlight_amd/csrc/kernels/fused_body.inc.h
+++ b/rustlight_amd/csrc/kernels/fused_body.inc.h
@@ -37,6 +37,7 @@
 #define RL_T0 { t0 = __builtin_readcyclecounter(); }
 #define RL_T1(K, COND) { unsigned long long t1 = __builtin_readcyclecounter(); tm[K] += t1 - t0; ln[K] += __popcll(__ballot(COND)); t0 = t1; }
     unsigned long long t0;
+    const unsigned long long wg_t0 = wall_clock64();
 #else
 #define RL_T0
 #define RL_T1(K, COND)
@@ -91,7 +92,12 @@
         ln[4] += 64;
         const bool c0 = PU(U_FLAGS) & ST_REGEN;
 #endif
-        if (PU(U_FLAGS) & ST_REGEN) raygen_slot<true, decltype(ps), SMP>(rc, sc, ps, n_samples, n_draws);
+#ifdef RL_FUSED_BODY_TAIL
+        constexpr bool kTail = RL_FUSED_BODY_TAIL;
+#else
+        constexpr bool kTail = false;
+#endif
+        if (PU(U_FLAGS) & ST_REGEN) raygen_slot<true, decltype(ps), SMP, kTail>(rc, sc, ps, n_samples, n_draws);
         RL_T1(0, c0)
 #ifdef RL_STAGE_TIMERS
         const bool c1 = PU(U_FLAGS) & ST_RAY;
@@ -125,3 +131,6 @@
         const unsigned vals[5] = {n_samples, n_vertices, n_draws, n_shadow, n_ext};
         block_stats<5>(rc.partials, which, vals);
     }
+#ifdef RL_STAGE_TIMERS
+    if (threadIdx.x == 0u && blockIdx.x < kFusedWgSlots) { g_fused_wgs[2 * blockIdx.x] = wg_t0; g_fused_wgs[2 * blockIdx.x + 1] = wall_clock64(); }
+#endif
diff --git a/rustlight_amd/csrc/kernels/knobs.h b/rustlight_amd/csrc/kernels/knobs.h
--- a/rustlight_amd/csrc/kernels/knobs.h
+++ b/rustlight_amd/csrc/kernels/knobs.h
@@ -16,6 +16,9 @@
     K_SPEC_DRAWS_PER_SAMPLE,
     K_ITEM_SHIFT,
     K_FUSED_DYNAMIC,
+    K_FUSED_TAIL_BLOCKS,
+    K_FUSED_TAIL_SPLIT,
+    K_FUSED_TAIL_NO_BUFFER_TEST,
     K_EVAL_SPLIT,
     K_EVAL_MIN, K_EVAL_DIV,
     K_NO_EVENTS,
@@ -40,7 +43,7 @@
     static const char* name_of(int k) {
         static const char* const names[K_COUNT] = {
             "ref_single_pass", "state_budget_mb", "no_overlap", "chain_serial", "chain_no_pre", "chain_no_treelets", "spec_force", "spec_draws_per_sample", "item_shift",
-            "fused_dynamic", "eval_split", "eval_min", "eval_div", "no_events", "queue_debug",
+            "fused_dynamic", "fused_tail_blocks", "fused_tail_split", "fused_tail_no_buffer_test", "eval_split", "eval_min", "eval_div", "no_events", "queue_debug",
             "spec_group", "spec_sub", "spec_cap", "spec_probe", "spec_lead", "spec_lead_max", "spec_lead_var", "spec_extra", "spec_dense", "spec_dense_frac",
             "spec_probe_every", "spec_ks", "spec_ke", "spec_serial_ratio", "spec_no_trivial", "spec_lds_limit_test", "spec_stats", "spec_wave_times", "spec_lds_levels", "vpl_batch_paths", "photon_tree_group_photons",
             "plane_generate_lanes", "plane_tree_device", "plane_tree_group_planes",
diff --git a/rustlight_amd/csrc/kernels/path_render.hip.h b/rustlight_amd/csrc/kernels/path_render.hip.h
--- a/rustlight_amd/csrc/kernels/path_render.hip.h
+++ b/rustlight_amd/csrc/kernels/path_render.hip.h
@@ -3,9 +3,12 @@
 namespace {
 
 using namespace rl;
+
+std::atomic<int> g_path_renders_in_flight{0};
 
 struct Plan { unsigned split, n_items, P, item_shift; };
 struct Chunk { unsigned c0, c1, n_pix; std::vector<unsigned> base; };
+struct Tail { unsigned begin, pixels, shift; };
 
 class PathRender : RenderFrame {
 public:
@@ -13,6 +16,7 @@
         : RenderFrame(c, seeds, nb, out, out_dev, stream_arg, s, p->shard_index, p->shard_count), params(p) {}
 
     int run() {
+        struct InFlight { InFlight() { g_path_renders_in_flight++; } ~InFlight() { g_path_renders_in_flight--; } } in_flight;
         int r;
         if ((r = choose_form()) != RL_OK) return r;
         plan_chunks();
@@ -36,6 +40,10 @@
     std::vector<Chunk> chunks;
     unsigned max_chunk_pix = 0;
     Plan plan{1u, 0u, 0u, 0u}, plan_chain{1u, 0u, 0u, 0u};
+    Tail tail{0u, 0u, 0u};
+    long long tail_blocks = 0;
+    unsigned tail_shift = 0;
+    bool tail_forced = false;
     unsigned split = 1, n_items = 0, item_shift = 0, P = 0, n_item_pixels = 0;
     Pool pool{};
     RenderConst rc{};
@@ -70,7 +78,9 @@
         return RL_OK;
     }
 
-    Plan plan_items(bool per_pixel, unsigned n_pix, unsigned n_chains) const {
+    bool dynamic_items() const { return knobs.has(K_FUSED_DYNAMIC) ? knobs.i(K_FUSED_DYNAMIC, 0) != 0 : (medium || !ctx->lds_scene); }
+
+    Plan plan_items(bool per_pixel, unsigned n_pix, unsigned n_chains, unsigned tail_lanes = 0u) const {
         Plan pl{1u, 0u, 0u, 0u};
         if (per_pixel && n_pix > 0) {
             const unsigned fused_groups = (n_pix + 255u) / 256u;
@@ -79,17 +89,17 @@
                                 : (fused ? (ctx->lds_scene ? fused_auto : std::max(fused_auto, 64u))
                                          : (ctx->lds_scene ? 1u : std::max(1u, (8u << 20) / std::max(1u, n_pix))));
             if (overlap_wanted && !params->sample_split) want = std::max(want, (unsigned)std::max<long long>(1, knobs.i(K_EVAL_SPLIT, 4)));
+            if (tail_forced) want = 1u;
             pl.split = std::max(1u, std::min(want, params->spp));
             if ((size_t)n_pix * params->spp * 3 * sizeof(float) > kSampleBufBudget || one_lane_per_pixel) pl.split = 1;
             while (pl.split > 1 && (size_t)n_pix * pl.split > (size_t)0x7fffff00u) pl.split--;
         }
-        pl.n_items = per_pixel ? n_pix * pl.split : n_chains;
+        pl.n_items = per_pixel ? n_pix * pl.split + tail_lanes : n_chains;
         unsigned Pp = params->pool_slots ? std::min(params->pool_slots, std::max(pl.n_items, 1u)) : std::min<unsigned>(pl.n_items, 16u << 20);
         Pp = std::max(256u, (unsigned)(((unsigned long long)Pp + 255ull) / 256ull * 256ull));
         if (fused) {
             const unsigned resident = (unsigned)cus * (unsigned)(ctx->lds_scene ? RL_FUSED_WAVES : RL_FUSED_WAVES_STREAMING) * 256u;
-            const bool dynamic_items = knobs.has(K_FUSED_DYNAMIC) ? knobs.i(K_FUSED_DYNAMIC, 0) != 0 : (medium || !ctx->lds_scene);
-            Pp = std::max(256u, (std::min(pl.n_items, dynamic_items ? resident : pl.n_items) + 255u) / 256u * 256u);
+            Pp = std::max(256u, (std::min(pl.n_items, dynamic_items() ? resident : pl.n_items) + 255u) / 256u * 256u);
             const unsigned resident4 = (unsigned)cus * 4u * 256u / ((medium && !per_pixel) ? 2u : 1u);
             while (pl.item_shift < 6u && ((size_t)pl.n_items << (pl.item_shift + 1u)) <= resident4) pl.item_shift++;
             if (!per_pixel && knobs.has(K_ITEM_SHIFT)) pl.item_shift = std::min(6u, (unsigned)std::max<long long>(0, knobs.i(K_ITEM_SHIFT, 0)));
@@ -133,6 +143,7 @@
     int plan_lanes() {
         overlap_wanted = two_pass && ctx->stream2 && !fast_math && !knobs.has(K_NO_OVERLAP) && knobs.i(K_SPEC_GROUP, 0) != 256;
         int rcode;
+        tail_request();
         for (int attempt = 0; attempt < 2; attempt++) {
             plan = two_pass ? plan_items(true, max_chunk_pix, 0) : plan_items(per_sample, n_pixels, (unsigned)owned.size());
             if (two_pass) for (const Chunk& ch : chunks) { const Plan pc = plan_items(true, ch.n_pix, 0); plan.P = std::max(plan.P, pc.P); plan.split = std::max(plan.split, pc.split); }
@@ -145,6 +156,7 @@
             if (params->sample_split || attempt == 1) return RL_ERR_HIP;
             one_lane_per_pixel = true; overlap_wanted = false;
         }
+        if ((rcode = plan_tail()) != RL_OK) return rcode;
         if ((rcode = alloc_tables()) != RL_OK) return rcode;
         if (per_sample || two_pass) {
             if (per_sample && (rcode = ctx->d_item_seed.ensure(n_item_pixels)) != RL_OK) return rcode;
@@ -164,6 +176,47 @@
         }
         pool = Pool{ctx->pool_f.get(), ctx->pool_u.get(), ctx->pool_q.get(), P};
         return alloc_output(std::max<size_t>((P + 255) / 256, (size_t)cus * 8u * rl_context::kEvalStreams));
+    }
+
+    static constexpr unsigned kFusedTailBlocks = 512u, kFusedTailSplit = 4u;
+    void tail_request() {
+        tail_blocks = 0; tail_shift = 0; tail_forced = false;
+        if (!per_sample || strat || two_pass || !fused || !ctx->lds_scene || medium || dynamic_items() || params->sample_split || owned.empty()) return;
+        const bool large = (n_pixels + 255u) / 256u >= 6000u && ctx->single_bsdf && ctx->bsdf_type == RL_BSDF_DIFFUSE && ctx->area_lights_only && !fast_math && g_path_renders_in_flight.load() <= 1;
+        const long long T = knobs.has(K_FUSED_TAIL_BLOCKS) ? knobs.i(K_FUSED_TAIL_BLOCKS, 0) : (large ? (long long)kFusedTailBlocks : 0);
+        const long long S = std::min<long long>(std::min<long long>(knobs.has(K_FUSED_TAIL_SPLIT) ? knobs.i(K_FUSED_TAIL_SPLIT, 0) : (long long)kFusedTailSplit, 64), params->spp);
+        unsigned shift = 0;
+        while ((2ll << shift) <= S) shift++;
+        if (T <= 0 || shift == 0u) return;
+        tail_blocks = T; tail_shift = shift;
+        tail_forced = knobs.has(K_FUSED_TAIL_BLOCKS) || knobs.has(K_FUSED_TAIL_SPLIT);
+    }
+    int plan_tail() {
+        tail = Tail{0u, 0u, 0u};
+        if (tail_blocks <= 0 || split != 1u) return RL_OK;
+        const long long T = tail_blocks;
+        const unsigned shift = tail_shift;
+        const bool expand = !params->has_max_depth || 1u < params->max_depth;
+        const uint64_t key = ((uint64_t)params->shard_index << 33) | ((uint64_t)shard_count << 1) | (expand ? 1u : 0u);
+        if (key != ctx->heavy_key || ctx->heavy_blocks.size() != owned.size()) {
+            std::vector<unsigned> masks;
+            trivial_pixel_masks(trivial_input(ctx), params, owned, nby, false, &masks, true);
+            ctx->heavy_blocks.assign(owned.size(), 0);
+            for (size_t j = 0; j < owned.size(); j++) ctx->heavy_blocks[j] = (masks[j * 8] & 1u) ? 0 : 1;
+            ctx->heavy_key = key;
+        }
+        size_t j0 = 0, j1 = 0; long long found = 0;
+        for (size_t j = owned.size(); j-- > 0 && found < T;) if (ctx->heavy_blocks[j]) { if (!found) j1 = j; j0 = j; found++; }
+        if (!found) return RL_OK;
+        const unsigned p0 = item_base[j0], p1 = j1 + 1 < owned.size() ? item_base[j1 + 1] : n_pixels;
+        const size_t lanes = (size_t)(p1 - p0) << shift;
+        if ((size_t)n_pixels + lanes > (size_t)0x7fffff00u || (size_t)(p1 - p0) * params->spp * 3 * sizeof(float) > kSampleBufBudget) return RL_OK;
+        if (knobs.has(K_FUSED_TAIL_NO_BUFFER_TEST) || ctx->d_sample_buf.ensure((size_t)(p1 - p0) * params->spp * 3) != RL_OK) { rl_set_error(""); return RL_OK; }
+        tail = Tail{p0, p1 - p0, shift};
+        plan = plan_items(true, n_pixels, 0, (unsigned)lanes - tail.pixels);
+        n_items = plan.n_items; item_shift = plan.item_shift;
+        P = std::max(plan.P, plan_chain.P);
+        return RL_OK;
     }
 
     int upload() {
@@ -183,6 +236,7 @@
         rc.n_items = n_items;
         rc.item_shift = item_shift;
         rc.split = split; rc.sample_buf = ctx->d_sample_buf.get();
+        rc.tail_begin = tail.begin; rc.tail_pixels = tail.pixels; rc.tail_shift = tail.shift; rc.tail_lanes = tail.pixels << tail.shift;
         rc.sample_states = ctx->d_sample_states.get(); rc.chain_states = ctx->d_chain_states.get();
 
         lds_trav = traversal_lds_bytes(ctx, ctx->lds_scene, 256, true);
@@ -545,6 +599,7 @@
 
     int finish() {
         if (split > 1 && !two_pass) { hipLaunchKernelGGL(k_fold_samples, dim3((n_pixels + 255) / 256), dim3(256), 0, st, rc); launches += 1; }
+        else if (tail.pixels) { hipLaunchKernelGGL(k_fold_samples, dim3((tail.pixels + 255) / 256), dim3(256), 0, st, rc); launches += 1; }
         const int rcode = download();
         if (rcode != RL_OK) return rcode;
         if (stats) {
diff --git a/rustlight_amd/csrc/kernels/pathstate.hip.h b/rustlight_amd/csrc/kernels/pathstate.hip.h
--- a/rustlight_amd/csrc/kernels/pathstate.hip.h
+++ b/rustlight_amd/csrc/kernels/pathstate.hip.h
@@ -124,6 +124,7 @@
     const unsigned* q_list;
     unsigned q_n;
     unsigned* q_ctr;
+    unsigned tail_begin, tail_lanes, tail_shift, tail_pixels;
 };
 RL_DEV void queue_workgroup_started(const RenderConst& rc) {
     if (atomicAdd(rc.queue, 1u) + 1u == rc.chain_grid) __hip_atomic_store(rc.started_flag, rc.queue_seq, __ATOMIC_RELEASE, __HIP_MEMORY_SCOPE_SYSTEM);
diff --git a/rustlight_amd/csrc/kernels/stages.hip.h b/rustlight_amd/csrc/kernels/stages.hip.h
--- a/rustlight_amd/csrc/kernels/stages.hip.h
+++ b/rustlight_amd/csrc/kernels/stages.hip.h
@@ -71,7 +71,7 @@
     PU(U_FLAGS) = ST_RAY | (PREV_SENSOR << ST_PREV_SHIFT) | ST_PDF_SA;
 }
 
-template <bool DYNAMIC, class PS, class SMP = Rng>
+template <bool DYNAMIC, class PS, class SMP = Rng, bool TAIL = false>
 RL_DEV void raygen_slot(const RenderConst& rc, const DeviceScene& sc, PS& ps, unsigned& n_samples, unsigned& n_draws) {
     unsigned flags = PU(U_FLAGS);
     if (!(flags & ST_REGEN)) return;
@@ -84,11 +84,23 @@
     constexpr bool STRAT = !std::is_same<SMP, Rng>::value;
     const bool per_pixel = STRAT || rc.stream_mode != RL_STREAM_REFERENCE_ORDER;
     const bool given = !STRAT && rc.stream_mode == kStreamGivenStates;
-    const unsigned split = per_pixel ? rc.split : 1u;
-    const unsigned pitem = split > 1u ? item / split : item;
+    unsigned split = per_pixel ? rc.split : 1u;
+    unsigned pitem = split > 1u ? item / split : item;
+    unsigned tail_begin = 0u, tail_lanes = 0u, tail_shift = 0u;
+    constexpr bool tail = TAIL;
+    if constexpr (TAIL) {
+        const char __attribute__((address_space(4)))* kt = (const char __attribute__((address_space(4)))*)__builtin_amdgcn_kernarg_segment_ptr();
+        asm volatile("" : "+s"(kt));
+        const RenderConst& rt = *(const RenderConst*)kt;
+        tail_begin = rt.tail_begin; tail_lanes = rt.tail_lanes; tail_shift = rt.tail_shift;
+        const unsigned rel = item - tail_begin;
+        const bool in_tail = rel < tail_lanes;
+        split = in_tail ? 1u << tail_shift : 1u;
+        pitem = in_tail ? tail_begin + (rel >> tail_shift) : (item < tail_begin ? item : item - (tail_lanes - (tail_lanes >> tail_shift)));
+    }
     if (!fresh && split > 1u) {
         const Col L = loadc(ps, F_LR);
-        float* dst = rc.sample_buf + 3 * ((size_t)s * (rc.n_items / split) + pitem);
+        float* dst = tail ? rc.sample_buf + 3 * ((size_t)s * (tail_lanes >> tail_shift) + (pitem - tail_begin)) : rc.sample_buf + 3 * ((size_t)s * (rc.n_items / split) + pitem);
         dst[0] = L.r; dst[1] = L.g; dst[2] = L.b;
         s += split;
         if (s >= rc.spp) need_item = true;
@@ -96,7 +108,7 @@
         acc = acc + loadc(ps, F_LR);
         s++;
         if (s == rc.spp) {
-            unsigned pix = per_pixel ? rc.item_pixel[item] : (by + cursor / bw) * rc.W + (bx + cursor % bw);
+            unsigned pix = per_pixel ? rc.item_pixel[TAIL ? pitem : item] : (by + cursor / bw) * rc.W + (bx + cursor % bw);
             Col px = scale_unguarded(acc, rc.inv_spp);
             rc.out[3 * (size_t)pix] = px.r; rc.out[3 * (size_t)pix + 1] = px.g; rc.out[3 * (size_t)pix + 2] = px.b;
             acc = czero();
@@ -119,9 +131,9 @@
             if (split > 1u) s = item % split;
             rng = load_sample_state(rc, s, pi);
         } else if (per_pixel) {
-            const unsigned pi = split > 1u ? item / split : item;
+            const unsigned pi = TAIL ? pitem : (split > 1u ? item / split : item);
             Rng item_rng = rng_seed(rc.item_seed[pi], rc.seed_variant);
-            if (split > 1u) { s = item % split; for (unsigned k = 0; k < s; k++) rng_next_u64(item_rng); }
+            if (split > 1u) { s = tail ? (item - tail_begin) & (split - 1u) : item % split; for (unsigned k = 0; k < s; k++) rng_next_u64(item_rng); }
             rng = rng_seed(rng_next_u64(item_rng), rc.seed_variant);
             store_rng(ps, Q_I0, item_rng);
         } else {
@@ -141,9 +153,9 @@
         rng = load_rng(ps, Q_R0);
     }
     unsigned px, py;
-    if (per_pixel) { unsigned pix = rc.item_pixel[split > 1u ? item / split : item]; px = pix % rc.W; py = pix / rc.W; }
+    if (per_pixel) { unsigned pix = rc.item_pixel[TAIL ? pitem : (split > 1u ? item / split : item)]; px = pix % rc.W; py = pix / rc.W; }
     else { px = bx + cursor % bw; py = by + cursor / bw; }
-    SMP smp = SmpState<SMP>::begin(rc, rng, split > 1u ? item / split : item, s);
+    SMP smp = SmpState<SMP>::begin(rc, rng, TAIL ? pitem : (split > 1u ? item / split : item), s);
     float u = (float)px + smp_next(smp);
     float v = (float)py + smp_next(smp);
     n_draws += 2;
diff --git a/rustlight_amd/csrc/kernels/wavefront.h b/rustlight_amd/csrc/kernels/wavefront.h
--- a/rustlight_amd/csrc/kernels/wavefront.h
+++ b/rustlight_amd/csrc/kernels/wavefront.h
@@ -20,6 +20,7 @@
 int rl_debug_rng_advance(int device, size_t n, const uint64_t* states_in, const uint32_t* counts, uint64_t* states_out);
 int rl_debug_stratified_draws(int device, size_t n_pixels, const uint64_t* pixel_seeds, uint32_t spp, int seed_variant, size_t n_calls, const int32_t* pattern, float* out);
 int rl_debug_trivial_pixels(const rl_scene* scene, int has_max_depth, uint32_t max_depth, uint8_t* out);
+int rl_debug_sample_buf_bytes(const rl_context* ctx, uint64_t* bytes);
 int rl_debug_bvh_sizes(const rl_context* ctx, uint64_t* n_ref_nodes, uint64_t* n_prims, uint32_t* stack_depth, int* lds_scene);
 int rl_debug_bvh(const rl_scene* scene, uint64_t* n_nodes, uint64_t* n_prims, float* boxes, uint64_t* info, uint64_t* count,
                  int32_t* prim_mesh, int32_t* prim_tri);
diff --git a/rustlight_amd/csrc/kernels/wavefront.hip b/rustlight_amd/csrc/kernels/wavefront.hip
--- a/rustlight_amd/csrc/kernels/wavefront.hip
+++ b/rustlight_amd/csrc/kernels/wavefront.hip
@@ -1,6 +1,7 @@
 #include <hip/hip_runtime.h>
 
 #include <algorithm>
+#include <atomic>
 #include <chrono>
 #include <cmath>
 #include <cstdio>
@@ -71,7 +72,8 @@
 }
 
 __global__ void __launch_bounds__(256) k_fold_samples(RenderConst rc) {
-    const unsigned n_pix = rc.n_items / rc.split;
+    const bool tail = rc.tail_lanes != 0u;
+    const unsigned n_pix = tail ? rc.tail_pixels : rc.n_items / rc.split;
     const unsigned p = blockIdx.x * blockDim.x + threadIdx.x;
     if (p >= n_pix) return;
     Col acc = czero();
@@ -80,7 +82,7 @@
         acc = acc + mkc(src[0], src[1], src[2]);
     }
     const Col px = scale_unguarded(acc, rc.inv_spp);
-    const size_t pix = rc.item_pixel[p];
+    const size_t pix = rc.item_pixel[tail ? rc.tail_begin + p : p];
     rc.out[3 * pix] = px.r; rc.out[3 * pix + 1] = px.g; rc.out[3 * pix + 2] = px.b;
 }
 
@@ -261,6 +263,8 @@
     HipBuffer<ulonglong2> d_trk_st;
     HipBuffer<unsigned> d_trivial;
     uint64_t trivial_key = ~0ull;
+    std::vector<unsigned char> heavy_blocks;
+    uint64_t heavy_key = ~0ull;
     HipBuffer<unsigned long long> d_spec_stats;
     std::vector<hipEvent_t> events;
     static constexpr int kEvalStreams = 4;
@@ -494,7 +498,7 @@
     in.camera = ctx->ds.camera;
     return in;
 }
-static void trivial_pixel_masks(const TrivialInput& ti, const rl_path_params* params, const std::vector<unsigned>& owned, size_t nby, bool no_shortcut, std::vector<unsigned>* out) {
+static void trivial_pixel_masks(const TrivialInput& ti, const rl_path_params* params, const std::vector<unsigned>& owned, size_t nby, bool no_shortcut, std::vector<unsigned>* out, bool blocks_only = false) {
     const uint32_t W = ti.W, H = ti.H;
     out->assign(owned.size() * 8, 0u);
     const bool expand = !params->has_max_depth || 1u < params->max_depth;
@@ -555,6 +559,7 @@
         const BlockRect r = block_rect(owned[j], nby, W, H);
         const unsigned bx = r.x, by = r.y, bw = r.w, bh = r.h;
         if (misses(bx - 0.25, by - 0.25, bx + bw + 0.25, by + bh + 0.25)) { all_of_block(j, bw * bh); continue; }
+        if (blocks_only) continue;
         for (unsigned c = 0; c < bw * bh; c++) {
             const double x = bx + c % bw, y = by + c / bw;
             if (misses(x - 0.25, y - 0.25, x + 1.25, y + 1.25)) (*out)[j * 8 + (c >> 5)] |= 1u << (c & 31u);
@@ -1299,6 +1304,11 @@
     return RL_OK;
 }
 
+extern "C" int rl_debug_sample_buf_bytes(const rl_context* ctx, uint64_t* bytes) {
+    if (!ctx || !bytes) return RL_ERR_INVALID_ARGUMENT;
+    *bytes = (uint64_t)ctx->d_sample_buf.capacity() * sizeof(float);
+    return RL_OK;
+}
 extern "C" int rl_debug_bvh_sizes(const rl_context* ctx, uint64_t* n_ref_nodes, uint64_t* n_prims, uint32_t* stack_depth, int* lds_scene) {
     if (!ctx) return RL_ERR_INVALID_ARGUMENT;
     *n_ref_nodes = ctx->bvh_dump.ref_info.size(); *n_prims = ctx->bvh_dump.ref_prim_mesh.size();
```
